# open-mmlab/PowerPaint

Hardware: AMD Instinct MI355X
Metric: inpainted images/sec @512x512, 50-step DDIM CFG, batch4/GPU (higher is better)
Workload: dtype bf16; 1 GPU; ppt-v1 SD1.5-inpaint UNet (9-ch in), 512x512, 50-step DDIM, CFG=7.5, bf16, batch=4/GPU; global_batch=4, denoise_steps=50, network_evaluations=50, parallelism=dp1 (image shards, no step collectives), hipgraph=True, weights=random init (no checkpoints offline)

## Files before the change

include/pp_hip.h:

```cpp
#ifndef PP_HIP_H_
#define PP_HIP_H_

#include <stddef.h>
#include <stdint.h>

#ifdef __cplusplus
extern "C" {
#endif

#define PP_OK 0
#define PP_ERR_BAD_ARG (-1)
#define PP_ERR_UNSUPPORTED (-2)
#define PP_ERR_LAUNCH (-3)
#define PP_ERR_WORKSPACE (-4)

#define PP_ABI_VERSION 29
#define PP_DT_F32 0
#define PP_DT_BF16 1
#define PP_DT_F16 2
int pp_abi_version(void);
const char* pp_build_id(void);
const char* pp_last_error(void);

#define PP_X_PLAIN 0
#define PP_X_CONV3X3 1
#define PP_ACT_NONE 0
#define PP_ACT_GEGLU 1
#define PP_ACT_SILU 2
#define PP_ACT_SOFTMAX80 3
#define PP_ACT_GELU 4

typedef struct PPGemmArgs {
  int32_t M, N, K;
  int32_t x_mode;
  const void* x1;
  const void* x2;
  int32_t c1, c2;
  int32_t ldx1, ldx2;
  int32_t batch, hin, win, hout, wout, stride, up;
  const void* w;
  const float* bias;
  const float* rowvec;
  int32_t ld_rowvec, rows_per_batch;
  const void* res1;
  int32_t ldres1;
  const void* res2;
  int32_t ldres2;
  float scale;
  int32_t act;
  void* out;
  int32_t ldo;
  int32_t out_f32;
  void* out_vt;
  int32_t vt_col0;
  int32_t vt_ld;
  int32_t splitk;
  int32_t tile;
  float* workspace;
  int32_t dbg;
  int32_t dtype;
  int32_t out_dup_rows;
  int32_t res1_wrap_rows;
  float* row_stats_out;
  const float* ln_stats;
  const float* ln_colsum;
  int32_t ln_tiles;
  int32_t ln_dim;
  float ln_eps;
  int32_t w_batch_stride;
  int64_t* gn_acc[2];
  int32_t gn_cg[2];
  int32_t gn_c0[2];
  int32_t gn_groups[2];
  const void* x3;
  const void* x4;
  int32_t c3;
  int32_t c4;
  const int64_t* gn_in_acc;
  const float* gn_in_gb;
  int32_t gn_in_groups;
  int32_t gn_in_silu;
  float gn_in_eps;
  int32_t gn_dup_batch;
  void* gn_next_out;
  const float* gn_next_gamma;
  const float* gn_next_beta;
  float gn_next_eps;
  int32_t gn_next_silu;
  int32_t gn_next_sub;
  int32_t gn_dup_mask;
  int32_t vec_batch_stride;
  uint64_t* tile_ctr;
  uint32_t* combine_fault;
  int32_t subpix;
  int32_t tile_group_m;
} PPGemmArgs;
#define PP_GN_SUM_SCALE 16777216.0f
#define PP_GN_SQ_SCALE 1048576.0f

#define PP_TILE_AUTO 0
#define PP_TILE_128x160 1
#define PP_TILE_64x160 2
#define PP_TILE_256x160 3

int pp_gemm_bf16(const PPGemmArgs* args, void* stream);
size_t pp_gemm_workspace_bytes(const PPGemmArgs* args);
int pp_gemm_gn_stats_ok(const PPGemmArgs* args);
int pp_conv_gn_supported(const PPGemmArgs* args);
int pp_conv_gn_preferred(const PPGemmArgs* args);
int pp_upconv_subpix_supported(int batch, int h, int w, int cin, int cout, int dtype);
int pp_upconv_subpix_supported_to(int batch, int h, int w, int hout, int wout, int cin, int cout, int dtype);
int pp_upconv_fold(const void* w, int cout, int cin, int dtype, void* out, void* stream);
int pp_gemm_gn_next_ok(const PPGemmArgs* args, int sub);
size_t pp_gemm_combine_ctr_bytes(const PPGemmArgs* args);
int pp_gemm_combine_fused(const PPGemmArgs* args);
int pp_gemm_tile_group_m(const PPGemmArgs* args);
int pp_xcd_placement_ok(void);

int pp_linear_skinny(const float* x, int rows, int K, const void* w, const float* bias, int N, float* out, int ldo,
                     int act_in, int act_out, int dtype, void* stream);

int pp_timestep_embedding(const float* t_dev, int rows, int dim, float* out, void* stream);

size_t pp_groupnorm_workspace_bytes(int batch, int hw, int C);
int pp_groupnorm_stats(const void* x1, int c1, const void* x2, int c2, int batch, int hw, int groups,
                       float* workspace, int dtype, void* stream);
int pp_groupnorm_apply(const void* x1, int c1, const void* x2, int c2, int batch, int hw, int groups, float eps,
                       const float* gamma, const float* beta, const float* workspace, int silu, void* y,
                       int dtype, void* stream);

int pp_groupnorm_apply_acc(const void* x1, int c1, const void* x2, int c2, int batch, int hw, int groups, float eps,
                           const float* gamma, const float* beta, const int64_t* acc, int silu, void* y, int dtype,
                           void* stream);
int pp_zero_u64(void* dst, long long n, void* stream);

int pp_layernorm(const void* x, int rows, int C, const float* gamma, const float* beta, float eps, void* y,
                 int dtype, void* stream);

int pp_attention_fwd(const void* q, int ldq, const void* k, int ldk, const void* vt, int ldvt, void* o, int ldo,
                     int batch, int heads, int nq, int nk, int d, float scale, int dtype, void* stream);
#define PP_ATTN_AUTO 0
#define PP_ATTN_PHASED 1
#define PP_ATTN_PIPE_Q32 2
#define PP_ATTN_PIPE_Q64 3
#define PP_ATTN_PIPE_LOG2 4
int pp_attention_log2_ok(int nq, int nk, int d);
int pp_attention_fwd_variant(const void* q, int ldq, const void* k, int ldk, const void* vt, int ldvt, void* o, int ldo,
                             int batch, int heads, int nq, int nk, int d, float scale, int dtype, int variant,
                             void* stream);
int pp_attention_tiled_ok(int h, int w, int nh, int nw, int d);
int pp_attention_fwd_tiled(const void* q, int ldq, const void* k, int ldk, const void* vt, int ldvt, void* o, int ldo,
                           int batch, int heads, int h, int w, int nh, int nw, int d, float scale, int variant,
                           int dtype, void* stream);
int pp_transpose_v(const void* v, int ld, int batch, int nk, int cols, void* vt, int ldvt, void* stream);

int pp_conv3x3_direct(const void* x, int batch, int hin, int win, int cin, const void* w, const float* bias,
                      int cout, int stride, int silu_out, const void* add, void* out, int dtype, void* stream);
int pp_conv3x3_smallcout(const void* x, int batch, int h, int w_, int cin, const void* w, const float* bias, int cout,
                         float* out_nchw, int dtype, void* stream);
int pp_gn_conv3x3_smallcout_supported(int cin, int cout, int groups);
int pp_gn_conv3x3_smallcout(const void* x, int batch, int h, int w, int cin, int groups, float eps, const float* gamma,
                            const float* beta, const int64_t* acc, const void* wgt, const float* bias, int cout,
                            float* out_nchw, int dtype, void* stream);

int pp_nchw_to_nhwc(const void* src, int src_dtype, int batch, int c, int hw, int src_batch_mod, void* dst, int ldc,
                    int c0, int dtype, void* stream);
int pp_nhwc_to_nchw(const void* src, int batch, int c, int hw, void* dst, int dst_dtype, int dtype, void* stream);
int pp_vit_patchify(const void* src, int src_dtype, int batch, int h, int w, int patch, void* dst, int cols, int ldo,
                    int dtype, void* stream);
int pp_vit_embed_ln(const void* patches, int ldp, const void* class_embedding, const void* pos, int batch, int np, int C,
                    const float* gamma, const float* beta, float eps, void* y, int dtype, void* stream);
int pp_add_bf16(const void* a, const void* b, void* out, long long n, int dtype, void* stream);

int pp_cfg_sched_step(const float* eps2, int cfg, float guidance, float* latents, float* m_prev, int n, int kind,
                      const float* coef_table, int32_t* step_dev, uint32_t* advance_ticket, void* stream);
int pp_ddim_variance_noise(float* latents, const float* noise, int n, const float* coef_table, const int32_t* step_dev,
                           void* stream);
int pp_cfg_lcm_step(const float* eps2, int cfg, float guidance, float* latents, const float* noise, int n,
                    const float* coef_table, int32_t* step_dev, uint32_t* advance_ticket, void* stream);
int pp_cfg_sigma_step(const float* eps2, int cfg, float guidance, float* latents, const float* noise, int n,
                      const float* coef_table, int32_t* step_dev, uint32_t* advance_ticket, void* stream);
int pp_cfg_ksampler_step(const float* eps2, int cfg, float guidance, float* latents, float* state, const float* noise, int n,
                         const float* coef_table, int32_t* step_dev, uint32_t* advance_ticket, void* stream);

int pp_tfront_supported(int M, int c, int rows_per_batch, int gn_groups);
int pp_tfront(const void* x, int ldx, const void* gn_acc, const float* gn_gamma, const float* gn_beta, float gn_eps, int gn_groups,
              const void* w1, const float* b1, const void* w2p, const float* cs2, const float* b2, float ln_eps, void* hs,
              int ldhs, void* qk, int ldqk, void* vt, int ldvt, int M, int c, int rows_per_batch, float q_scale, int dtype,
              void* stream);
int pp_xattn_block_supported(int M, int c, int rows_per_batch, int nctx, int heads);
int pp_xattn_fold(const void* k, int ldk, const void* vt, int ldvt, int batch, int nctx, int heads, int c, const void* wq,
                  const float* q_colsum, const float* q_bias, const void* wo, float scale, void* gt, float* gcs,
                  float* gbias, void* ht, int kperm, int dtype, void* stream);
int pp_xattn_block(const void* x, int ldx, const void* res, int ldres, const float* ln_stats, int ln_tiles, float ln_eps,
                   const void* gt, const float* gcs, const float* gbias, const void* ht, const float* bias_o, void* out,
                   int ldo, float* row_stats_out, int M, int c, int rows_per_batch, int src_wrap_rows, const void* pre_w,
                   const float* pre_b, int dtype, void* stream);

int pp_ff_fused_supported(int M, int c, int rows_per_batch);
int pp_ff_fused(const PPGemmArgs* g2, const void* w1, const float* b1, const float* cs1, const float* ln_stats, int ln_tiles,
                float ln_eps, int w2_kperm, void* stream);

int pp_latent_blend(float* latents, const float* image_latents, const float* mask, const float* noise,
                    const float* renoise_table, const int32_t* step_dev, int batch, int channels, int hw, void* stream);

int pp_step_head(const float* temb_table, const int32_t* step_dev, float* temb_out, int row_floats, const float* latents,
                 int batch, int c, int hw, int src_batch_mod, void* x_in, int ldc, int c0, int dtype, void* zero_dst,
                 long long n_zero, void* stream);
int pp_step_head_scaled(const float* temb_table, const int32_t* step_dev, float* temb_out, int row_floats, const float* latents,
                        int batch, int c, int hw, int src_batch_mod, void* x_in, int ldc, int c0, int dtype, void* zero_dst,
                        long long n_zero, const float* in_div, void* stream);
int pp_step_select_t(const float* timesteps, const int32_t* step_dev, float* t_out, void* stream);
int pp_step_advance(int32_t* step_dev, void* stream);

int pp_mask_prep(int mode, const float* a, const float* b, float* out, int batch, int c, int h, int w, int ho, int wo,
                 void* stream);

int pp_embed_splice(const void* table, const void* ext, const int32_t* src_row, void* out, int n_rows,
                    long long row_bytes, void* stream);

int pp_softmax_rows(const float* s, long long lds, int rows, int n, float scale, void* p, long long ldp, int dtype,
                    void* stream);

int pp_attention_small(const void* q, int ldq, const void* k, int ldk, const void* v, int ldv, void* o, int ldo,
                       int batch, int heads, int nq, int nk, int d, float scale, int causal, int dtype, void* stream);

#define PP_LORA_MAX_ADAPTERS 8
#define PP_LORA_MAX_RANK 128
#define PP_LORA_ROWS_PLAIN 0
#define PP_LORA_ROWS_GEGLU 1
#define PP_LORA_COLS_PLAIN 0
#define PP_LORA_COLS_IGEMM 1
#define PP_LORA_COLS_KPERM 2
#define PP_LORA_COLS_KPERM_GEGLU 3
typedef struct PPLoraMergeArgs {
  int32_t N, K;
  const float* w;
  int64_t ldw;
  int32_t n_adapters;
  int32_t rank[PP_LORA_MAX_ADAPTERS];
  float coef[PP_LORA_MAX_ADAPTERS];
  const float* up[PP_LORA_MAX_ADAPTERS];
  const float* down[PP_LORA_MAX_ADAPTERS];
  const float* gamma;
  const float* beta;
  const float* badd;
  void* out;
  int64_t ldo;
  int32_t out_rows, out_cols, out_dtype;
  int32_t row_mode, row_off;
  int32_t col_mode, col_off, taps, cin_pad;
  float* colsum;
  float* bias;
} PPLoraMergeArgs;
int pp_lora_merge(const PPLoraMergeArgs* args, void* stream);

int pp_freeu(const void* hidden, void* hidden_out, int ch, const void* skip, void* skip_out, int cs, int batch, int h, int w,
             const float* bs, int64_t* acc, int groups, int dtype, void* stream);

#define PP_IP_MAX_TOKENS 64
int pp_ip_attn_add(const void* q, int ldq, const void* k_ip, const void* v_ip, void* o, int ldo, int batch, int heads, int nq,
                   int nk, int d, float qk_scale, float ip_scale, int dtype, void* stream);

int pp_ip_attn_add_masked(const void* q, int ldq, const void* k_ip, const void* v_ip, void* o, int ldo, int batch, int heads,
                          int nq, int nk, int d, float qk_scale, float ip_scale, const float* row_w, int dtype, void* stream);

int pp_perceiver_attn(const void* q, int ldq, const void* kv_x, int ldkx, int nx, const void* kv_l, int ldkl, int nl, void* o,
                      int ldo, int batch, int heads, int nq, int d, float scale, int dtype, void* stream);

#define PP_TOME_MAX_TOKENS 16384
int pp_tome_supported(int h, int w, int C, int sx, int sy);
int pp_tome_match(const void* x, int ldx, int batch, int h, int w, int C, int sx, int sy, const void* table,
                  int table_row_stride, int table_rows, const void* row_idx, void* best_dst, void* score, int dtype,
                  void* stream);
int pp_tome_select(const void* best_dst, const void* score, int batch, int n, int nd, int r, void* pos, void* rowtok, void* seg,
                   void* lst, void* stream);
int pp_tome_merge(const void* qk, int ldqk, const void* vt, int ldvt, int batch, int n, int C, int nd, int r, const void* rowtok,
                  const void* seg, const void* lst, void* qk_out, int ldqk_out, void* vt_out, int ldvt_out, int dtype,
                  void* stream);
int pp_tome_unmerge(const void* a, int lda, const void* pos, int batch, int n, int nm, int C, void* out, int ldo, void* stream);

int pp_attn_identity_v(const void* vt, int ldvt, int batch0, int batch, int n, int C, void* out, int ldo, void* stream);
int pp_pag_combine(float* eps, int cfg, float guidance, const float* pag_table, const int32_t* step_dev, int n, void* stream);

int pp_cfg_rescale(float* eps, int segs, float guidance, const float* pag_table, const float* phi_dev, const int32_t* step_dev,
                   int batch, int per, void* stream);

int pp_conv4x4s2(const void* x, int batch, int hin, int win, int cin, const void* w, const float* bias, int cout, int relu_in,
                 void* out, int dtype, void* stream);
int pp_relu(const void* x, void* out, long long n, int dtype, void* stream);
int pp_masked_image_pack(const float* image, const float* mask, int batch, int c, int h, int w, void* out, int dtype,
                         void* stream);
int pp_mask_blend(const void* sample, const void* cond, const float* mask, void* out, int batch, int h, int w, int c,
                  int mask_h, int mask_w, int64_t* acc, int groups, int dtype, void* stream);

#ifdef __cplusplus
}
#endif
#endif
```

powerpaint_amd/_lib.py:

```python
import ctypes as C
import os

_HERE = os.path.dirname(os.path.abspath(__file__))
LIB_PATH = os.path.join(_HERE, "libpp_hip.so")
if os.environ.get("PP_LAB") == "1" and os.environ.get("PP_LIB"):
    LIB_PATH = os.path.abspath(os.environ["PP_LIB"])

PP_X_PLAIN, PP_X_CONV3X3 = 0, 1
PP_ACT_NONE, PP_ACT_GEGLU, PP_ACT_SILU, PP_ACT_SOFTMAX80, PP_ACT_GELU = 0, 1, 2, 3, 4
PP_TILE_AUTO, PP_TILE_128x160, PP_TILE_64x160, PP_TILE_256x160 = 0, 1, 2, 3
PP_DT_F32, PP_DT_BF16, PP_DT_F16 = 0, 1, 2
PP_ATTN_AUTO, PP_ATTN_PHASED, PP_ATTN_PIPE_Q32, PP_ATTN_PIPE_Q64, PP_ATTN_PIPE_LOG2 = 0, 1, 2, 3, 4
ABI_VERSION = 29
PP_ERR = {0: "PP_OK", -1: "PP_ERR_BAD_ARG", -2: "PP_ERR_UNSUPPORTED", -3: "PP_ERR_LAUNCH", -4: "PP_ERR_WORKSPACE"}

vp, i32, f32, sz = C.c_void_p, C.c_int32, C.c_float, C.c_size_t


class PPGemmArgs(C.Structure):
    _fields_ = [
        ("M", i32), ("N", i32), ("K", i32), ("x_mode", i32),
        ("x1", vp), ("x2", vp),
        ("c1", i32), ("c2", i32), ("ldx1", i32), ("ldx2", i32),
        ("batch", i32), ("hin", i32), ("win", i32), ("hout", i32), ("wout", i32), ("stride", i32), ("up", i32),
        ("w", vp), ("bias", vp), ("rowvec", vp),
        ("ld_rowvec", i32), ("rows_per_batch", i32),
        ("res1", vp), ("ldres1", i32),
        ("res2", vp), ("ldres2", i32),
        ("scale", f32), ("act", i32),
        ("out", vp), ("ldo", i32), ("out_f32", i32),
        ("out_vt", vp), ("vt_col0", i32), ("vt_ld", i32),
        ("splitk", i32), ("tile", i32),
        ("workspace", vp),
        ("dbg", i32), ("dtype", i32), ("out_dup_rows", i32), ("res1_wrap_rows", i32),
        ("row_stats_out", vp), ("ln_stats", vp), ("ln_colsum", vp),
        ("ln_tiles", i32), ("ln_dim", i32), ("ln_eps", f32), ("w_batch_stride", i32),
        ("gn_acc", vp * 2), ("gn_cg", i32 * 2), ("gn_c0", i32 * 2), ("gn_groups", i32 * 2),
        ("x3", vp), ("x4", vp), ("c3", i32), ("c4", i32),
        ("gn_in_acc", vp), ("gn_in_gb", vp), ("gn_in_groups", i32), ("gn_in_silu", i32), ("gn_in_eps", f32),
        ("gn_dup_batch", i32),
        ("gn_next_out", vp), ("gn_next_gamma", vp), ("gn_next_beta", vp), ("gn_next_eps", f32), ("gn_next_silu", i32),
        ("gn_next_sub", i32), ("gn_dup_mask", i32), ("vec_batch_stride", i32),
        ("tile_ctr", vp), ("combine_fault", vp),
        ("subpix", i32),
        ("tile_group_m", i32),
    ]


def gemm_args(dtype: int, M: int, N: int, K: int, x, w, out, x2=None, K2: int = 0, ldx=None, ldx2: int = 0, ldo: int = 0,
              ldres1: int = 0, ldres2: int = 0, rows_per_batch: int = 0, scale: float = 1.0) -> PPGemmArgs:
    a = PPGemmArgs()
    a.dtype = dtype
    a.M, a.N, a.K, a.x_mode = M, N, K + K2, PP_X_PLAIN
    a.x1, a.x2, a.c1, a.c2 = x, x2 or None, K, K2
    a.ldx1, a.ldx2 = (K if ldx is None else ldx), (ldx2 or K2)
    a.w, a.out = w, out
    a.ldo, a.ldres1, a.ldres2 = ldo or N, ldres1 or N, ldres2 or N
    a.rows_per_batch, a.scale = rows_per_batch, scale
    return a


def conv3x3_args(dtype: int, B: int, H: int, W: int, c1: int, cout: int, x, x2=None, c2: int = 0, x3=None, c3: int = 0,
                 x4=None, c4: int = 0, stride: int = 1, up: bool = False, w=None, out=None, scale: float = 1.0,
                 up_size=None) -> PPGemmArgs:
    hv, wv = (2 * H, 2 * W) if up else (H, W)
    if up_size is not None:
        if not up or stride != 1 or up_size[0] not in (2 * H - 1, 2 * H) or up_size[1] not in (2 * W - 1, 2 * W):
            raise ValueError(f"up_size {tuple(up_size)} is no nearest-resize target of a {H}x{W} source")
        hv, wv = up_size
    ho, wo = (hv - 1) // stride + 1, (wv - 1) // stride + 1
    a = PPGemmArgs()
    a.dtype = dtype
    a.M, a.N, a.K, a.x_mode = B * ho * wo, cout, 9 * (c1 + c2) + c3 + c4, PP_X_CONV3X3
    a.x1, a.x2, a.c1, a.c2 = x, x2 or None, c1, c2
    a.x3, a.x4, a.c3, a.c4 = x3 or None, x4 or None, c3, c4
    a.batch, a.hin, a.win, a.hout, a.wout, a.stride, a.up = B, H, W, ho, wo, stride, int(up)
    a.w, a.out = w, out
    a.ldo, a.ldres1, a.ldres2 = cout, cout, cout
    a.rows_per_batch, a.scale = ho * wo, scale
    return a


PP_LORA_MAX_ADAPTERS, PP_LORA_MAX_RANK = 8, 128
PP_LORA_ROWS_PLAIN, PP_LORA_ROWS_GEGLU = 0, 1
PP_TOME_MAX_TOKENS = 16384
PP_IP_MAX_TOKENS = 64
PP_LORA_COLS_PLAIN, PP_LORA_COLS_IGEMM, PP_LORA_COLS_KPERM, PP_LORA_COLS_KPERM_GEGLU = 0, 1, 2, 3


class PPLoraMergeArgs(C.Structure):
    _fields_ = [
        ("N", i32), ("K", i32), ("w", vp), ("ldw", C.c_int64), ("n_adapters", i32),
        ("rank", i32 * PP_LORA_MAX_ADAPTERS), ("coef", f32 * PP_LORA_MAX_ADAPTERS),
        ("up", vp * PP_LORA_MAX_ADAPTERS), ("down", vp * PP_LORA_MAX_ADAPTERS),
        ("gamma", vp), ("beta", vp), ("badd", vp),
        ("out", vp), ("ldo", C.c_int64), ("out_rows", i32), ("out_cols", i32), ("out_dtype", i32),
        ("row_mode", i32), ("row_off", i32), ("col_mode", i32), ("col_off", i32), ("taps", i32), ("cin_pad", i32),
        ("colsum", vp), ("bias", vp),
    ]


SIGNATURES = {
    "pp_abi_version": (C.c_int, []),
    "pp_last_error": (C.c_char_p, []),
    "pp_build_id": (C.c_char_p, []),
    "pp_gemm_bf16": (C.c_int, [C.POINTER(PPGemmArgs), vp]),
    "pp_gemm_workspace_bytes": (sz, [C.POINTER(PPGemmArgs)]),
    "pp_linear_skinny": (C.c_int, [vp, C.c_int, C.c_int, vp, vp, C.c_int, vp, C.c_int, C.c_int, C.c_int, C.c_int, vp]),
    "pp_timestep_embedding": (C.c_int, [vp, C.c_int, C.c_int, vp, vp]),
    "pp_groupnorm_workspace_bytes": (sz, [C.c_int, C.c_int, C.c_int]),
    "pp_gemm_gn_stats_ok": (C.c_int, [C.POINTER(PPGemmArgs)]),
    "pp_conv_gn_supported": (C.c_int, [C.POINTER(PPGemmArgs)]),
    "pp_conv_gn_preferred": (C.c_int, [C.POINTER(PPGemmArgs)]),
    "pp_gemm_gn_next_ok": (C.c_int, [C.POINTER(PPGemmArgs), C.c_int]),
    "pp_upconv_subpix_supported": (C.c_int, [C.c_int] * 6),
    "pp_upconv_subpix_supported_to": (C.c_int, [C.c_int] * 8),
    "pp_upconv_fold": (C.c_int, [vp, C.c_int, C.c_int, C.c_int, vp, vp]),
    "pp_gemm_combine_ctr_bytes": (sz, [C.POINTER(PPGemmArgs)]),
    "pp_gemm_combine_fused": (C.c_int, [C.POINTER(PPGemmArgs)]),
    "pp_gemm_tile_group_m": (C.c_int, [C.POINTER(PPGemmArgs)]),
    "pp_xcd_placement_ok": (C.c_int, []),
    "pp_groupnorm_apply_acc": (C.c_int, [vp, C.c_int, vp, C.c_int, C.c_int, C.c_int, C.c_int, f32, vp, vp, vp, C.c_int, vp,
                                         C.c_int, vp]),
    "pp_zero_u64": (C.c_int, [vp, C.c_longlong, vp]),
    "pp_embed_splice": (C.c_int, [vp, vp, vp, vp, C.c_int, C.c_longlong, vp]),
    "pp_attention_small": (C.c_int, [vp, C.c_int, vp, C.c_int, vp, C.c_int, vp, C.c_int, C.c_int, C.c_int, C.c_int,
                                     C.c_int, C.c_int, f32, C.c_int, C.c_int, vp]),
    "pp_softmax_rows": (C.c_int, [vp, C.c_longlong, C.c_int, C.c_int, f32, vp, C.c_longlong, C.c_int, vp]),
    "pp_groupnorm_stats": (C.c_int, [vp, C.c_int, vp, C.c_int, C.c_int, C.c_int, C.c_int, vp, C.c_int, vp]),
    "pp_groupnorm_apply": (C.c_int, [vp, C.c_int, vp, C.c_int, C.c_int, C.c_int, C.c_int, f32, vp, vp, vp, C.c_int, vp,
                                     C.c_int, vp]),
    "pp_layernorm": (C.c_int, [vp, C.c_int, C.c_int, vp, vp, f32, vp, C.c_int, vp]),
    "pp_attention_fwd": (C.c_int, [vp, C.c_int, vp, C.c_int, vp, C.c_int, vp, C.c_int, C.c_int, C.c_int, C.c_int,
                                   C.c_int, C.c_int, f32, C.c_int, vp]),
    "pp_attention_fwd_variant": (C.c_int, [vp, C.c_int, vp, C.c_int, vp, C.c_int, vp, C.c_int, C.c_int, C.c_int, C.c_int,
                                           C.c_int, C.c_int, f32, C.c_int, C.c_int, vp]),
    "pp_attention_tiled_ok": (C.c_int, [C.c_int] * 5),
    "pp_attention_fwd_tiled": (C.c_int, [vp, C.c_int, vp, C.c_int, vp, C.c_int, vp, C.c_int, C.c_int, C.c_int, C.c_int,
                                         C.c_int, C.c_int, C.c_int, C.c_int, f32, C.c_int, C.c_int, vp]),
    "pp_transpose_v": (C.c_int, [vp, C.c_int, C.c_int, C.c_int, C.c_int, vp, C.c_int, vp]),
    "pp_conv3x3_direct": (C.c_int, [vp, C.c_int, C.c_int, C.c_int, C.c_int, vp, vp, C.c_int, C.c_int, C.c_int, vp,
                                    vp, C.c_int, vp]),
    "pp_conv3x3_smallcout": (C.c_int, [vp, C.c_int, C.c_int, C.c_int, C.c_int, vp, vp, C.c_int, vp, C.c_int, vp]),
    "pp_nchw_to_nhwc": (C.c_int, [vp, C.c_int, C.c_int, C.c_int, C.c_int, C.c_int, vp, C.c_int, C.c_int, C.c_int, vp]),
    "pp_nhwc_to_nchw": (C.c_int, [vp, C.c_int, C.c_int, C.c_int, vp, C.c_int, C.c_int, vp]),
    "pp_vit_patchify": (C.c_int, [vp, C.c_int, C.c_int, C.c_int, C.c_int, C.c_int, vp, C.c_int, C.c_int, C.c_int, vp]),
    "pp_vit_embed_ln": (C.c_int, [vp, C.c_int, vp, vp, C.c_int, C.c_int, C.c_int, vp, vp, f32, vp, C.c_int, vp]),
    "pp_add_bf16": (C.c_int, [vp, vp, vp, C.c_longlong, C.c_int, vp]),
    "pp_cfg_sched_step": (C.c_int, [vp, C.c_int, f32, vp, vp, C.c_int, C.c_int, vp, vp, vp, vp]),
    "pp_step_select_t": (C.c_int, [vp, vp, vp, vp]),
    "pp_ddim_variance_noise": (C.c_int, [vp, vp, C.c_int, vp, vp, vp]),
    "pp_cfg_lcm_step": (C.c_int, [vp, C.c_int, f32, vp, vp, C.c_int, vp, vp, vp, vp]),
    "pp_cfg_sigma_step": (C.c_int, [vp, C.c_int, f32, vp, vp, C.c_int, vp, vp, vp, vp]),
    "pp_cfg_ksampler_step": (C.c_int, [vp, C.c_int, f32, vp, vp, vp, C.c_int, vp, vp, vp, vp]),
    "pp_latent_blend": (C.c_int, [vp, vp, vp, vp, vp, vp, C.c_int, C.c_int, C.c_int, vp]),
    "pp_gn_conv3x3_smallcout_supported": (C.c_int, [C.c_int] * 3),
    "pp_gn_conv3x3_smallcout": (C.c_int, [vp, C.c_int, C.c_int, C.c_int, C.c_int, C.c_int, C.c_float, vp, vp, vp, vp, vp,
                                          C.c_int, vp, C.c_int, vp]),
    "pp_tfront_supported": (C.c_int, [C.c_int] * 4),
    "pp_tfront": (C.c_int, [vp, C.c_int, vp, vp, vp, C.c_float, C.c_int, vp, vp, vp, vp, vp, C.c_float, vp, C.c_int, vp, C.c_int,
                            vp, C.c_int, C.c_int, C.c_int, C.c_int, C.c_float, C.c_int, vp]),
    "pp_attention_log2_ok": (C.c_int, [C.c_int] * 3),
    "pp_xattn_block_supported": (C.c_int, [C.c_int] * 5),
    "pp_xattn_fold": (C.c_int, [vp, C.c_int, vp, C.c_int, C.c_int, C.c_int, C.c_int, C.c_int, vp, vp, vp, vp, C.c_float,
                                vp, vp, vp, vp, C.c_int, C.c_int, vp]),
    "pp_xattn_block": (C.c_int, [vp, C.c_int, vp, C.c_int, vp, C.c_int, C.c_float, vp, vp, vp, vp, vp, vp, C.c_int, vp,
                                 C.c_int, C.c_int, C.c_int, C.c_int, vp, vp, C.c_int, vp]),
    "pp_ff_fused_supported": (C.c_int, [C.c_int] * 3),
    "pp_ff_fused": (C.c_int, [C.POINTER(PPGemmArgs), vp, vp, vp, vp, C.c_int, C.c_float, C.c_int, vp]),
    "pp_step_head": (C.c_int, [vp, vp, vp, C.c_int, vp, C.c_int, C.c_int, C.c_int, C.c_int, vp, C.c_int, C.c_int, C.c_int, vp,
                              C.c_longlong, vp]),
    "pp_step_head_scaled": (C.c_int, [vp, vp, vp, C.c_int, vp, C.c_int, C.c_int, C.c_int, C.c_int, vp, C.c_int, C.c_int, C.c_int,
                                     vp, C.c_longlong, vp, vp]),
    "pp_step_advance": (C.c_int, [vp, vp]),
    "pp_lora_merge": (C.c_int, [C.POINTER(PPLoraMergeArgs), vp]),
    "pp_freeu": (C.c_int, [vp, vp, C.c_int, vp, vp, C.c_int, C.c_int, C.c_int, C.c_int, vp, vp, C.c_int, C.c_int, vp]),
    "pp_mask_prep": (C.c_int, [C.c_int, vp, vp, vp, C.c_int, C.c_int, C.c_int, C.c_int, C.c_int, C.c_int, vp]),
    "pp_ip_attn_add": (C.c_int, [vp, C.c_int, vp, vp, vp, C.c_int, C.c_int, C.c_int, C.c_int, C.c_int, C.c_int, f32, f32,
                                 C.c_int, vp]),
    "pp_ip_attn_add_masked": (C.c_int, [vp, C.c_int, vp, vp, vp, C.c_int, C.c_int, C.c_int, C.c_int, C.c_int, C.c_int, f32, f32,
                                        vp, C.c_int, vp]),
    "pp_perceiver_attn": (C.c_int, [vp, C.c_int, vp, C.c_int, C.c_int, vp, C.c_int, C.c_int, vp, C.c_int, C.c_int, C.c_int,
                                    C.c_int, C.c_int, f32, C.c_int, vp]),
    "pp_tome_supported": (C.c_int, [C.c_int] * 5),
    "pp_tome_match": (C.c_int, [vp, C.c_int, C.c_int, C.c_int, C.c_int, C.c_int, C.c_int, C.c_int, vp, C.c_int, C.c_int, vp, vp,
                                vp, C.c_int, vp]),
    "pp_tome_select": (C.c_int, [vp, vp, C.c_int, C.c_int, C.c_int, C.c_int, vp, vp, vp, vp, vp]),
    "pp_tome_merge": (C.c_int, [vp, C.c_int, vp, C.c_int, C.c_int, C.c_int, C.c_int, C.c_int, C.c_int, vp, vp, vp, vp, C.c_int,
                                vp, C.c_int, C.c_int, vp]),
    "pp_tome_unmerge": (C.c_int, [vp, C.c_int, vp, C.c_int, C.c_int, C.c_int, C.c_int, vp, C.c_int, vp]),
    "pp_attn_identity_v": (C.c_int, [vp, C.c_int, C.c_int, C.c_int, C.c_int, C.c_int, vp, C.c_int, vp]),
    "pp_pag_combine": (C.c_int, [vp, C.c_int, f32, vp, vp, C.c_int, vp]),
    "pp_cfg_rescale": (C.c_int, [vp, C.c_int, f32, vp, vp, vp, C.c_int, C.c_int, vp]),
    "pp_conv4x4s2": (C.c_int, [vp, C.c_int, C.c_int, C.c_int, C.c_int, vp, vp, C.c_int, C.c_int, vp, C.c_int, vp]),
    "pp_relu": (C.c_int, [vp, vp, C.c_longlong, C.c_int, vp]),
    "pp_masked_image_pack": (C.c_int, [vp, vp, C.c_int, C.c_int, C.c_int, C.c_int, vp, C.c_int, vp]),
    "pp_mask_blend": (C.c_int, [vp, vp, vp, vp, C.c_int, C.c_int, C.c_int, C.c_int, C.c_int, C.c_int, vp, C.c_int, C.c_int, vp]),
}

_lib = None


class PPError(RuntimeError):
    pass


def lib():
    global _lib
    if _lib is None:
        if not os.path.exists(LIB_PATH):
            raise PPError(
                f"{LIB_PATH} not found: the HIP extension is not built. Run `python -c 'import __graft_entry__ as g; "
                f"g.build()'` (or `make -C powerpaint_amd/csrc`). There is no CPU/PyTorch fallback.")
        l = C.CDLL(LIB_PATH)
        for name, (res, args) in SIGNATURES.items():
            fn = getattr(l, name)
            fn.restype = res
            fn.argtypes = args
        if l.pp_abi_version() != ABI_VERSION:
            raise PPError("libpp_hip.so ABI version mismatch")
        _lib = l
    return _lib


def dtype_code(dtype) -> int:
    import torch
    if dtype == torch.bfloat16:
        return PP_DT_BF16
    if dtype == torch.float16:
        return PP_DT_F16
    raise PPError(f"the HIP path computes in bf16 or fp16 (fp32 accumulate), not {dtype}")


def build_id() -> str:
    return lib().pp_build_id().decode()


def check(rc: int, what: str = ""):
    if rc != 0:
        msg = lib().pp_last_error().decode() if rc == -3 else ""
        raise PPError(f"{what} failed: {PP_ERR.get(rc, rc)} {msg}")
```

powerpaint_amd/csrc/conv_gn.hip:

```cpp
#include <type_traits>
#include <utility>

#include "pp_common.h"
#include "gemm_gn.h"
#include "gemm_combine.h"

namespace {

typedef __attribute__((address_space(3))) void* cg_lds_t;

constexpr int CG_T = 512, CG_BN = 160, CG_NI = 5;
constexpr int CG_WP = 3;
constexpr int CG_HPW_MAX = 6;
constexpr int CG_HALO_PX = 384;
constexpr int CG_HALO = CG_HALO_PX * 128;
constexpr int CG_WST = CG_BN * 128;
constexpr int CG_WOFF = 2 * CG_HALO;
constexpr int CG_TAB = CG_WOFF + 3 * CG_WST;
constexpr int CG_T_STATS = CG_TAB;
constexpr int CG_T_ZERO = CG_TAB + 256;
constexpr int CG_T_GB = CG_TAB + 1024;
constexpr int CG_T_SCSH = CG_TAB + 3072;
constexpr int CG_LDS = CG_TAB + 3584;
static_assert(CG_LDS <= 160 * 1024, "LDS budget");

struct CGDerived {
  int tiles_m, tiles_n, group_m;
  int nch1, nch;
  int ntail3, ntail;
  int hp;
  int cg;
  float inv_cg;
};

template <int... I, class F>
PP_DEVINL void cg_static_for_impl(std::integer_sequence<int, I...>, F&& f) { (f(std::integral_constant<int, I>{}), ...); }
template <int N, class F>
PP_DEVINL void cg_static_for(F&& f) { cg_static_for_impl(std::make_integer_sequence<int, N>{}, f); }

template <int BM, int HPW, bool PP, int NMODE, int EDT>
__global__ void __launch_bounds__(CG_T, 2) pp_conv_gn_kernel(const PPGemmArgs a, const CGDerived d) {
  using E = E16<EDT>;
  typedef typename E::v8 v8_t;
  constexpr int T = CG_T, WN = 2, MI = BM / 64, NI = CG_NI, BN = CG_BN;
  constexpr int CG_HPW = HPW;
  constexpr bool SUBPIX = NMODE == 4;
  static_assert(!SUBPIX || PP, "the sub-pixel form has the ping-pong loop only");
  constexpr bool NORM = NMODE != 2 && !SUBPIX;
  constexpr bool NREAD = NMODE == 0 || NMODE == 3;
  static_assert(HPW >= 2 && HPW <= CG_HPW_MAX, "halo strips per wave");
  constexpr int XP2 = BM / 64;
  constexpr int P2 = XP2 + CG_WP;
  constexpr int ST2 = BM * 128;
  constexpr int EPI_ROWS = 64, EPI_LD = BN * 4 + 16;
  constexpr int RS_OFF = EPI_ROWS * EPI_LD + BM * 8;
  static_assert(3 * ST2 <= 2 * CG_HALO, "tail stages live in the halo buffers");
  static_assert(MI * 16 <= EPI_ROWS && EPI_ROWS % (MI * 16) == 0, "wave rows vs epilogue pass");

  extern __shared__ __attribute__((aligned(16))) char smem[];

  const int tid = threadIdx.x;
  const int lane = tid & 63;
  const int wave = __builtin_amdgcn_readfirstlane(tid >> 6);
  const int wm = wave >> 1, wn = wave & 1;
  const int grp = wave >> 2;

  int lid;
  {
    const int nwg = gridDim.x, bid = blockIdx.x;
    const int q = nwg >> 3, r = nwg & 7, xcd = bid & 7, idx = bid >> 3;
    lid = (xcd < r ? xcd * (q + 1) : r * (q + 1) + (xcd - r) * q) + idx;
  }
  const int par = SUBPIX ? (lid & 3) : 0, pa = par >> 1, pb = par & 1;
  if constexpr (SUBPIX) lid >>= 2;
  int tile_m, tile_n;
  pp_tile_decode(lid, d.tiles_m, d.tiles_n, d.group_m, &tile_m, &tile_n);
  const int m_blk = tile_m * BM, n_blk = tile_n * BN;
  const int split = blockIdx.y, splits = gridDim.y;
  const int ch_b = split * d.nch / splits, ch_e = (split + 1) * d.nch / splits;
  const int tk_b = split * d.ntail / splits, tk_e = (split + 1) * d.ntail / splits;

  const int Wd = a.wout, Hd = a.hout, HW = Hd * Wd;
  const int HWs = a.hin * a.win;
  const int bimg = m_blk / HW;
  const int y0 = (m_blk - bimg * HW) / Wd;
  const int ctot = a.c1 + a.c2;
  const uint32_t wbytes = (uint32_t)a.N * (uint32_t)a.K * 2u;
  const void* const wmat = SUBPIX ? (const void*)((const char*)a.w + (size_t)par * wbytes) : a.w;

  const int lrow = lane >> 3;
  const int kslot = (lane & 7) ^ lrow;

  int vw[CG_WP], wlds[CG_WP];
#pragma unroll
  for (int i = 0; i < CG_WP; ++i) {
    const int strip = (wave * 8 + i * 64 < BN) ? i : i - 1;
    const int n = n_blk + wave * 8 + lrow + strip * 64;
    vw[i] = (n < a.N) ? (n * a.K + kslot * 8) * 2 : (int)PP_OOB;
    wlds[i] = (wave * 8 + strip * 64) * 128;
  }
  int hpix[CG_HPW];
#pragma unroll
  for (int j = 0; j < CG_HPW; ++j) {
    const int hp = (wave + 8 * j) * 8 + lrow;
    const int hr = hp / Wd, hx = hp - hr * Wd;
    const int iy = y0 + hr - 1;
    hpix[j] = (hp < d.hp && iy >= 0 && iy < Hd) ? (a.up ? bimg * HWs + (iy >> 1) * a.win + (hx >> 1) : bimg * HW + iy * Wd + hx) : -1;
  }
  const int r16 = lane & 15, g = lane >> 4;
  const int fsw = r16 & 7;
  const int wrow0 = wn * (NI * 16) + r16;
  const int rt0 = wm * (MI * 16) + r16;
  unsigned edge = 0u;
#pragma unroll
  for (int mi = 0; mi < MI; ++mi) {
    const int lx = (rt0 + mi * 16) % Wd;
    if (lx == 0) edge |= 1u << mi;
    if (lx == Wd - 1) edge |= 1u << (8 + mi);
  }

  f32x4_t acc[NI][MI];
#pragma unroll
  for (int ni = 0; ni < NI; ++ni)
#pragma unroll
    for (int mi = 0; mi < MI; ++mi) acc[ni][mi] = f32x4_t{0.f, 0.f, 0.f, 0.f};

  auto mfma_all = [&](const v8_t (&wf)[2][NI], const v8_t (&xf)[2][MI]) __attribute__((always_inline)) {
#pragma unroll
    for (int ks = 0; ks < 2; ++ks)
#pragma unroll
      for (int ni = 0; ni < NI; ++ni)
#pragma unroll
        for (int mi = 0; mi < MI; ++mi) acc[ni][mi] = E::mfma16(wf[ks][ni], xf[ks][mi], acc[ni][mi]);
  };

  if (ch_b < ch_e) {
    auto issue_gb = [&](int c, int gbuf, bool live) __attribute__((always_inline)) {
      const __amdgpu_buffer_rsrc_t rs = make_rsrc(a.gn_in_gb, (NORM && live) ? (uint32_t)ctot * 8u : 0u);
      const int vo = lane < 32 ? lane * 16 : (int)PP_OOB;
      __builtin_amdgcn_raw_ptr_buffer_load_lds(rs, (cg_lds_t)(smem + CG_T_GB + gbuf * 1024), 16, vo, c * 512, 0, 0);
    };
    auto compute_scsh = [&](int c, int gbuf) __attribute__((always_inline)) {
      const char* gp = smem + CG_T_GB + gbuf * 1024 + kslot * 64;
      const f32x2_t* st = reinterpret_cast<const f32x2_t*>(smem + CG_T_STATS);
#pragma unroll
      for (int q = 0; q < 4; ++q) {
        const f32x4_t gbv = *reinterpret_cast<const f32x4_t*>(gp + q * 16);
        f32x4_t o;
#pragma unroll
        for (int h = 0; h < 2; ++h) {
          const int ch = c * 64 + kslot * 8 + 2 * q + h;
          const int gi = min((int)(((float)ch + 0.5f) * d.inv_cg), 31);
          const f32x2_t mr = st[gi];
          const float sv = mr[1] * gbv[2 * h];
          o[2 * h] = sv;
          o[2 * h + 1] = gbv[2 * h + 1] - mr[0] * sv;
        }
        if (lrow == 0) *reinterpret_cast<f32x4_t*>(smem + CG_T_SCSH + kslot * 64 + q * 16) = o;
      }
      asm volatile("s_waitcnt lgkmcnt(0)" ::: "memory");
    };
    auto norm_piece = [&](int hbuf, int j) __attribute__((always_inline)) {
      char* p = smem + hbuf * CG_HALO + (wave + 8 * j) * 1024 + lane * 16;
      if (hpix[j] >= 0) {
        const u32x4_t v = *reinterpret_cast<const u32x4_t*>(p);
        float r[8];
#pragma unroll
        for (int q = 0; q < 4; ++q) {
          const f32x4_t ss = *reinterpret_cast<const f32x4_t*>(smem + CG_T_SCSH + kslot * 64 + q * 16);
          r[2 * q] = E::lo(v[q]) * ss[0] + ss[1];
          r[2 * q + 1] = E::hi(v[q]) * ss[2] + ss[3];
        }
#pragma unroll
        for (int e = 0; e < 8; ++e)
          r[e] = r[e] * __builtin_amdgcn_rcpf(1.0f + __builtin_amdgcn_exp2f(r[e] * -1.44269504088896340736f));
        u32x4_t o;
#pragma unroll
        for (int q = 0; q < 4; ++q) o[q] = E::pack2(r[2 * q], r[2 * q + 1]);
        *reinterpret_cast<u32x4_t*>(p) = o;
      }
    };

    auto norm_math = [&](const u32x4_t v, uint32_t vmask) __attribute__((always_inline)) -> u32x4_t {
      u32x4_t o;
#pragma unroll
      for (int q = 0; q < 4; ++q) {
        const f32x4_t ss = *reinterpret_cast<const f32x4_t*>(smem + CG_T_SCSH + kslot * 64 + q * 16);
        float r0 = E::lo(v[q]) * ss[0] + ss[1];
        float r1 = E::hi(v[q]) * ss[2] + ss[3];
        const float e0 = __builtin_amdgcn_exp2f(r0 * -1.44269504088896340736f);
        const float e1 = __builtin_amdgcn_exp2f(r1 * -1.44269504088896340736f);
        r0 *= __builtin_amdgcn_rcpf(1.0f + e0);
        r1 *= __builtin_amdgcn_rcpf(1.0f + e1);
        o[q] = E::pack2(r0, r1) & vmask;
      }
      return o;
    };

    __amdgpu_buffer_rsrc_t rs_h = make_rsrc(a.x1, 0u);
    int hsoff = 0, hcsrc = 0;
    auto halo_source = [&](int c, bool live) __attribute__((always_inline)) {
      const bool first = c < d.nch1;
      int csrc;
      if (first) {
        csrc = a.c1;
        rs_h = make_rsrc(a.x1, live ? (uint32_t)a.batch * (uint32_t)HWs * (uint32_t)a.c1 * 2u : 0u);
        hsoff = c * 128;
      } else {
        csrc = a.c2;
        rs_h = make_rsrc(a.x2 ? a.x2 : a.x1, (live && a.x2) ? (uint32_t)a.batch * (uint32_t)HWs * (uint32_t)a.c2 * 2u : 0u);
        hsoff = (c - d.nch1) * 128;
      }
      hcsrc = csrc;
    };
    auto issue_halo_piece = [&](int hbuf, int j) __attribute__((always_inline)) {
      const int vo = hpix[j] >= 0 ? (hpix[j] * hcsrc + kslot * 8) * 2 : (int)PP_OOB;
      __builtin_amdgcn_raw_ptr_buffer_load_lds(rs_h, (cg_lds_t)(smem + hbuf * CG_HALO + (wave + 8 * j) * 1024), 16, vo,
                                               hsoff, 0, 0);
    };
    auto issue_w_piece = [&](const __amdgpu_buffer_rsrc_t rs, int stage, int i, int sow) __attribute__((always_inline)) {
      const int vo = vw[i], lo = wlds[i];
      __builtin_amdgcn_raw_ptr_buffer_load_lds(rs, (cg_lds_t)(smem + CG_WOFF + stage * CG_WST + lo), 16, vo, sow, 0, 0);
    };

    {
      const __amdgpu_buffer_rsrc_t rsw = make_rsrc(wmat, wbytes);
#pragma unroll
      for (int i = 0; i < CG_WP; ++i) issue_w_piece(rsw, 0, i, (0 * ctot + ch_b * 64) * 2);
#pragma unroll
      for (int i = 0; i < CG_WP; ++i) issue_w_piece(rsw, 1, i, (1 * ctot + ch_b * 64) * 2);
      halo_source(ch_b, true);
#pragma unroll
      for (int j = 0; j < CG_HPW; ++j) issue_halo_piece(0, j);
      issue_gb(ch_b, 0, true);
    }
    if (NORM && tid < a.gn_in_groups) {
      const long long* ap = reinterpret_cast<const long long*>(a.gn_in_acc) + ((size_t)bimg * a.gn_in_groups + tid) * 2;
      const double s = (double)ap[0] * (1.0 / (double)PP_GN_SUM_SCALE);
      const double q = (double)ap[1] * (1.0 / (double)PP_GN_SQ_SCALE);
      const double n = (double)HW * (double)d.cg;
      const double mean = s / n;
      double var = q / n - mean * mean;
      if (var < 0.0) var = 0.0;
      reinterpret_cast<f32x2_t*>(smem + CG_T_STATS)[tid] = f32x2_t{(float)mean, (float)(1.0 / sqrt(var + (double)a.gn_in_eps))};
    }
    if (tid < 32) reinterpret_cast<float*>(smem + CG_T_ZERO)[tid] = 0.f;
    asm volatile("s_waitcnt vmcnt(0) lgkmcnt(0)\n\ts_barrier" ::: "memory");
    if constexpr (NORM) {
      compute_scsh(ch_b, 0);
#pragma unroll
      for (int j = 0; j < CG_HPW; ++j) norm_piece(0, j);
    }
    asm volatile("s_waitcnt lgkmcnt(0)\n\ts_barrier" ::: "memory");
    if (PP && grp == 1) asm volatile("s_barrier" ::: "memory");

    int hb = 0;
    if constexpr (SUBPIX) {
      int st = 0;
      const int tap00 = pa * Wd + pb - 1;
      const unsigned em0 = pb == 0 ? (edge & 0xffu) : 0u, em1 = pb == 1 ? (edge >> 8) : 0u;
#pragma unroll 1
      for (int c = ch_b; c < ch_e; ++c) {
        const bool nxt = c + 1 < ch_e;
        halo_source(c + 1, nxt);
        const __amdgpu_buffer_rsrc_t rsw_same = make_rsrc(wmat, wbytes);
        const __amdgpu_buffer_rsrc_t rsw_next = make_rsrc(wmat, nxt ? wbytes : 0u);
        const int hoff = hb * CG_HALO;
        const int hbn = hb ^ 1;
        int Wl = Wd;
        asm volatile("" : "+s"(Wl));

        cg_static_for<4>([&](auto TT) __attribute__((always_inline)) {
          constexpr int t = decltype(TT)::value;
          constexpr auto NXT = [](int tt) constexpr { return tt > 2 ? 0 : (2 * tt + 2 <= CG_HPW ? 2 : 2 * tt + 1 <= CG_HPW ? 1 : 0); };
          constexpr int NX = NXT(t);
          const int st_w = st == 0 ? 2 : st - 1;
          const __amdgpu_buffer_rsrc_t rsw = t + 2 <= 3 ? rsw_same : rsw_next;
          const int sow = t + 2 <= 3 ? ((t + 2) * ctot + c * 64) * 2 : ((t + 2 - 4) * ctot + (c + 1) * 64) * 2;

          asm volatile("s_barrier" ::: "memory");
          const char* ws = smem + CG_WOFF + st * CG_WST;
          const int hp0 = rt0 + tap00 + (t / 2) * Wl + (t % 2);
          const int xbase = hoff + (hp0 << 7) + ((g ^ (hp0 & 7)) << 4);
          const unsigned em = t % 2 == 0 ? em0 : em1;
          v8_t wf[2][NI], xf[2][MI];
          constexpr int NR = NI + MI, NPC = CG_WP + NX;
#pragma unroll
          for (int r = 0; r < NR; ++r) {
            if (r < NI) {
              const int ni = r < NI ? r : 0;
              const char* pw = ws + (wrow0 + ni * 16) * 128;
              wf[0][ni] = *reinterpret_cast<const v8_t*>(pw + ((g ^ fsw) << 4));
              wf[1][ni] = *reinterpret_cast<const v8_t*>(pw + (((4 + g) ^ fsw) << 4));
            } else {
              const int mi = r >= NI ? r - NI : 0;
              int o0 = xbase + mi * 2048;
              o0 = (em >> mi) & 1u ? CG_T_ZERO : o0;
              xf[0][mi] = *reinterpret_cast<const v8_t*>(smem + o0);
              xf[1][mi] = *reinterpret_cast<const v8_t*>(smem + (o0 ^ 64));
            }
#pragma unroll
            for (int k = 0; k < NPC; ++k)
              if (((k + 1) * NR + NPC) / (NPC + 1) == r + 1) {
                __builtin_amdgcn_sched_barrier(0);
                if (k < CG_WP) issue_w_piece(rsw, st_w, k < CG_WP ? k : 0, sow);
                else issue_halo_piece(hbn, 2 * t + (k - CG_WP < 2 ? k - CG_WP : 0));
                __builtin_amdgcn_sched_barrier(0);
              }
          }
          constexpr int V = (t == 3 ? 0 : NXT((t + 3) % 4)) + CG_WP + NX;
          asm volatile("s_waitcnt vmcnt(%0) lgkmcnt(0)\n\ts_barrier" ::"n"(V) : "memory");
          __builtin_amdgcn_sched_barrier(0);
          __builtin_amdgcn_s_setprio(1);
          mfma_all(wf, xf);
          __builtin_amdgcn_s_setprio(0);
          __builtin_amdgcn_sched_barrier(0);
          st = st == 2 ? 0 : st + 1;
        });
        hb ^= 1;
      }
    } else {
  #pragma unroll 1
      for (int c = ch_b; c < ch_e; ++c) {
        const bool nxt = c + 1 < ch_e;
        halo_source(c + 1, nxt);
        const __amdgpu_buffer_rsrc_t rsw_same = make_rsrc(wmat, wbytes);
        const __amdgpu_buffer_rsrc_t rsw_next = make_rsrc(wmat, nxt ? wbytes : 0u);
        const int hoff = hb * CG_HALO;
        const int hbn = hb ^ 1;
        int Wl = Wd;
        asm volatile("" : "+s"(Wl));

        cg_static_for<9>([&](auto TT) __attribute__((always_inline)) {
          constexpr int t = decltype(TT)::value;
          constexpr int st_r = t % 3, st_w = (t + 2) % 3;
          constexpr auto NXT = [](int tt) constexpr {
            const int nh = tt > 2 ? 0 : (2 * tt + 2 <= CG_HPW ? 2 : 2 * tt + 1 <= CG_HPW ? 1 : 0);
            return nh + (tt == 0 ? 1 : 0);
          };
          constexpr int NX = NXT(t);
          const __amdgpu_buffer_rsrc_t rsw = t + 2 <= 8 ? rsw_same : rsw_next;
          const int sow = t + 2 <= 8 ? ((t + 2) * ctot + c * 64) * 2 : ((t + 2 - 9) * ctot + (c + 1) * 64) * 2;

          if constexpr (PP) {
            asm volatile("s_barrier" ::: "memory");
          } else {
            constexpr int V = NXT((t + 7) % 9) + CG_WP + NXT((t + 8) % 9);
            asm volatile("s_waitcnt vmcnt(%0) lgkmcnt(0)\n\ts_barrier" ::"n"(V) : "memory");
          }
          constexpr bool NT = NORM && t >= 3 && t - 3 < CG_HPW;
          char* const np = smem + hbn * CG_HALO + (wave + 8 * (NT ? t - 3 : 0)) * 1024 + lane * 16;
          u32x4_t nv = {0u, 0u, 0u, 0u};
          f32x4_t ss0 = {0.f, 0.f, 0.f, 0.f}, ss1 = {0.f, 0.f, 0.f, 0.f};
          if constexpr (NT) {
            if constexpr (t == 3) compute_scsh(c + 1, hbn);
            if constexpr (NREAD) norm_piece(hbn, t - 3);
            else {
              nv = *reinterpret_cast<const u32x4_t*>(np);
              ss0 = *reinterpret_cast<const f32x4_t*>(smem + CG_T_SCSH + kslot * 64);
              ss1 = *reinterpret_cast<const f32x4_t*>(smem + CG_T_SCSH + kslot * 64 + 16);
            }
            if constexpr (NREAD) __builtin_amdgcn_sched_barrier(0);
          }
          const char* ws = smem + CG_WOFF + st_r * CG_WST;
          const int hp0 = rt0 + (t / 3) * Wl + (t % 3) - 1;
          const int xbase = hoff + (hp0 << 7) + ((g ^ (hp0 & 7)) << 4);
          v8_t wf[2][NI], xf[2][MI];
          constexpr int NR = NI + MI, NPC = CG_WP + NX;
  #pragma unroll
          for (int r = 0; r < NR; ++r) {
            if (r < NI) {
              const int ni = r < NI ? r : 0;
              const char* pw = ws + (wrow0 + ni * 16) * 128;
              wf[0][ni] = *reinterpret_cast<const v8_t*>(pw + ((g ^ fsw) << 4));
              wf[1][ni] = *reinterpret_cast<const v8_t*>(pw + (((4 + g) ^ fsw) << 4));
            } else {
              const int mi = r >= NI ? r - NI : 0;
              int o0 = xbase + mi * 2048;
              if constexpr (t % 3 == 0) o0 = (edge >> mi) & 1u ? CG_T_ZERO : o0;
              if constexpr (t % 3 == 2) o0 = (edge >> (8 + mi)) & 1u ? CG_T_ZERO : o0;
              xf[0][mi] = *reinterpret_cast<const v8_t*>(smem + o0);
              xf[1][mi] = *reinterpret_cast<const v8_t*>(smem + (o0 ^ 64));
            }
  #pragma unroll
            for (int k = 0; k < NPC; ++k)
              if (((k + 1) * NR + NPC) / (NPC + 1) == r + 1) {
                __builtin_amdgcn_sched_barrier(0);
                if (k < CG_WP) issue_w_piece(rsw, st_w, k < CG_WP ? k : 0, sow);
                else if (t == 0 && k == NPC - 1) issue_gb(c + 1, hbn, nxt);
                else issue_halo_piece(hbn, 2 * t + (k - CG_WP < 2 ? k - CG_WP : 0));
                __builtin_amdgcn_sched_barrier(0);
              }
          }
          if constexpr (PP) {
            constexpr int V = NXT((t + 8) % 9) + CG_WP + NX;
            asm volatile("s_waitcnt vmcnt(%0) lgkmcnt(0)\n\ts_barrier" ::"n"(V) : "memory");
          }
          __builtin_amdgcn_sched_barrier(0);
          if constexpr (NMODE != 3) __builtin_amdgcn_s_setprio(1);
          if constexpr (NT && NMODE == 1) {
            constexpr int NM = 2 * MI * NI, NG = 41;
            const uint32_t vmask = ~(uint32_t)(hpix[NT ? t - 3 : 0] >> 31);
            const char* const sp = smem + CG_T_SCSH + kslot * 64;
            float xa[4], ea[4];
            u32x4_t no;
            auto micro = [&](auto GG) __attribute__((always_inline)) {
              constexpr int g = decltype(GG)::value;
              if constexpr (g == 40) {
                *reinterpret_cast<u32x4_t*>(np) = no;
              } else {
                constexpr int h = g / 20, gg = g % 20, p0 = 2 * h, p1 = 2 * h + 1;
                if constexpr (gg == 0) { xa[0] = E::lo(nv[p0]); xa[1] = E::hi(nv[p0]); }
                if constexpr (gg == 1) { xa[2] = E::lo(nv[p1]); xa[3] = E::hi(nv[p1]); }
                if constexpr (gg == 2) { xa[0] = __builtin_fmaf(xa[0], ss0[0], ss0[1]); xa[1] = __builtin_fmaf(xa[1], ss0[2], ss0[3]); }
                if constexpr (gg == 3) { xa[2] = __builtin_fmaf(xa[2], ss1[0], ss1[1]); xa[3] = __builtin_fmaf(xa[3], ss1[2], ss1[3]); }
                if constexpr (gg == 4) { ea[0] = xa[0] * -1.44269504088896340736f; ea[1] = xa[1] * -1.44269504088896340736f; }
                if constexpr (gg == 5) { ea[2] = xa[2] * -1.44269504088896340736f; ea[3] = xa[3] * -1.44269504088896340736f; }
                if constexpr (gg == 6) {
                  ea[0] = __builtin_amdgcn_exp2f(ea[0]);
                  if constexpr (h == 0) ss0 = *reinterpret_cast<const f32x4_t*>(sp + 32);
                }
                if constexpr (gg == 7) {
                  ea[1] = __builtin_amdgcn_exp2f(ea[1]);
                  if constexpr (h == 0) ss1 = *reinterpret_cast<const f32x4_t*>(sp + 48);
                }
                if constexpr (gg == 8) ea[2] = __builtin_amdgcn_exp2f(ea[2]);
                if constexpr (gg == 9) ea[3] = __builtin_amdgcn_exp2f(ea[3]);
                if constexpr (gg == 10) { ea[0] += 1.0f; ea[1] += 1.0f; }
                if constexpr (gg == 11) { ea[2] += 1.0f; ea[3] += 1.0f; }
                if constexpr (gg == 12) ea[0] = __builtin_amdgcn_rcpf(ea[0]);
                if constexpr (gg == 13) ea[1] = __builtin_amdgcn_rcpf(ea[1]);
                if constexpr (gg == 14) ea[2] = __builtin_amdgcn_rcpf(ea[2]);
                if constexpr (gg == 15) ea[3] = __builtin_amdgcn_rcpf(ea[3]);
                if constexpr (gg == 16) { xa[0] *= ea[0]; xa[1] *= ea[1]; }
                if constexpr (gg == 17) { xa[2] *= ea[2]; xa[3] *= ea[3]; }
                if constexpr (gg == 18) no[p0] = E::pack2(xa[0], xa[1]) & vmask;
                if constexpr (gg == 19) no[p1] = E::pack2(xa[2], xa[3]) & vmask;
              }
            };
            cg_static_for<NM>([&](auto II) __attribute__((always_inline)) {
              constexpr int i = decltype(II)::value;
              constexpr int ks = i / (NI * MI), ni = (i / MI) % NI, mi = i % MI;
              acc[ni][mi] = E::mfma16(wf[ks][ni], xf[ks][mi], acc[ni][mi]);
              __builtin_amdgcn_sched_barrier(0);
              constexpr int G0 = i * NG / NM, G1 = (i + 1) * NG / NM;
              cg_static_for<G1 - G0>([&](auto JJ) __attribute__((always_inline)) {
                micro(std::integral_constant<int, G0 + decltype(JJ)::value>{});
              });
              __builtin_amdgcn_sched_barrier(0);
            });
          } else {
            mfma_all(wf, xf);
          }
          if constexpr (NMODE != 3) __builtin_amdgcn_s_setprio(0);
          __builtin_amdgcn_sched_barrier(0);
        });
        hb ^= 1;
      }
    }
    if (PP && grp == 0) asm volatile("s_barrier" ::: "memory");
    asm volatile("s_waitcnt vmcnt(0)" ::: "memory");
  }

  if (tk_b < tk_e) {
    asm volatile("s_waitcnt lgkmcnt(0)\n\ts_barrier" ::: "memory");
    const int mrow = m_blk + wave * 8 + lrow;
    const uint32_t xb3 = (uint32_t)a.M * (uint32_t)a.c3 * 2u, xb4 = a.x4 ? (uint32_t)a.M * (uint32_t)a.c4 * 2u : 0u;
    auto issue2 = [&](int kt, int stage) __attribute__((always_inline)) {
      const bool live = kt < tk_e;
      const bool first = kt < d.ntail3;
      const __amdgpu_buffer_rsrc_t rsx = first ? make_rsrc(a.x3, live ? xb3 : 0u) : make_rsrc(a.x4 ? a.x4 : a.x3, live ? xb4 : 0u);
      const int sox = (first ? kt : kt - d.ntail3) * 128;
      const int csrc = first ? a.c3 : a.c4;
      const __amdgpu_buffer_rsrc_t rsw = make_rsrc(a.w, live ? wbytes : 0u);
      const int sow = (9 * ctot + kt * 64) * 2;
#pragma unroll
      for (int i = 0; i < XP2; ++i) {
        const int m = mrow + i * 64;
        const int vo = m < a.M ? (m * csrc + kslot * 8) * 2 : (int)PP_OOB;
        __builtin_amdgcn_raw_ptr_buffer_load_lds(rsx, (cg_lds_t)(smem + stage * ST2 + (wave * 8 + i * 64) * 128), 16, vo, sox,
                                                 0, 0);
      }
#pragma unroll
      for (int i = 0; i < CG_WP; ++i) {
        const int vo = vw[i], lo = wlds[i];
        __builtin_amdgcn_raw_ptr_buffer_load_lds(rsw, (cg_lds_t)(smem + CG_WOFF + stage * CG_WST + lo), 16, vo, sow, 0, 0);
      }
    };
    issue2(tk_b, 0);
    issue2(tk_b + 1, 1);
    const int xrow0 = wm * (MI * 16) + r16;
    int stage = 0;
#pragma unroll 1
    for (int kt = tk_b; kt < tk_e; ++kt) {
      asm volatile("s_waitcnt vmcnt(%0)\n\ts_barrier" ::"n"(P2) : "memory");
      int nstage = stage + 2;
      if (nstage >= 3) nstage -= 3;
      issue2(kt + 2, nstage);
      const char* xs = smem + stage * ST2;
      const char* ws = smem + CG_WOFF + stage * CG_WST;
      v8_t wf[2][NI], xf[2][MI];
#pragma unroll
      for (int ks = 0; ks < 2; ++ks) {
        const int so = ((ks * 4 + g) ^ fsw) << 4;
#pragma unroll
        for (int ni = 0; ni < NI; ++ni) wf[ks][ni] = *reinterpret_cast<const v8_t*>(ws + (wrow0 + ni * 16) * 128 + so);
#pragma unroll
        for (int mi = 0; mi < MI; ++mi) xf[ks][mi] = *reinterpret_cast<const v8_t*>(xs + (xrow0 + mi * 16) * 128 + so);
      }
      __builtin_amdgcn_sched_barrier(0);
      __builtin_amdgcn_s_setprio(1);
      mfma_all(wf, xf);
      __builtin_amdgcn_s_setprio(0);
      stage = stage + 1 == 3 ? 0 : stage + 1;
    }
    asm volatile("s_waitcnt vmcnt(0)" ::: "memory");
  }

  auto out_row = [&](int m) __attribute__((always_inline)) -> size_t {
    const int l = m - bimg * HW, i = l / Wd, j = l - i * Wd;
    return (size_t)bimg * 4u * (size_t)HW + (size_t)((2 * i + pa) * 2 * Wd + 2 * j + pb);
  };
  const bool splitk = splits > 1;
  const bool gns = !splitk && (a.gn_acc[0] || a.gn_acc[1]);
  const int my_pass = (wm * (MI * 16)) / EPI_ROWS;
  const int my_row0 = (wm * (MI * 16)) % EPI_ROWS;
  float gcs[8], gcq[8];
#pragma unroll
  for (int jj = 0; jj < 8; ++jj) { gcs[jj] = 0.f; gcq[jj] = 0.f; }
  constexpr int EC = BN / 8, ER = T / EC, EP = (EPI_ROWS + ER - 1) / ER;
  const int c8 = tid % EC, r0 = tid / EC;
  const int n = n_blk + c8 * 8;
#pragma unroll 1
  for (int pass = 0; pass < BM / EPI_ROWS; ++pass) {
    asm volatile("s_waitcnt lgkmcnt(0)\n\ts_barrier" ::: "memory");
    if (my_pass == pass) {
#pragma unroll
      for (int mi = 0; mi < MI; ++mi)
#pragma unroll
        for (int ni = 0; ni < NI; ++ni)
          *reinterpret_cast<f32x4_t*>(smem + (my_row0 + mi * 16 + r16) * EPI_LD + (wn * (NI * 16) + ni * 16 + 4 * g) * 4) =
              acc[ni][mi];
    }
    asm volatile("s_waitcnt lgkmcnt(0)\n\ts_barrier" ::: "memory");
    const int m0 = m_blk + pass * EPI_ROWS;
    if (r0 < ER && n < a.N) {
      if (splitk) {
#pragma unroll
        for (int j = 0; j < EP; ++j) {
          const int row = r0 + j * ER, m = m0 + row;
          if (row < EPI_ROWS && m < a.M) {
            float* wsp = a.workspace + ((size_t)split * a.M + m) * a.N + n;
            *reinterpret_cast<f32x4_t*>(wsp) = *reinterpret_cast<const f32x4_t*>(smem + row * EPI_LD + c8 * 32);
            *reinterpret_cast<f32x4_t*>(wsp + 4) = *reinterpret_cast<const f32x4_t*>(smem + row * EPI_LD + c8 * 32 + 16);
          }
        }
      } else {
        u32x4_t r1[EP], r2[EP];
#pragma unroll
        for (int j = 0; j < EP; ++j) {
          const int row = r0 + j * ER, m = m0 + row;
          const bool ok = row < EPI_ROWS && m < a.M;
          const size_t m1 = SUBPIX ? out_row(m) : (size_t)((a.res1_wrap_rows > 0 && m >= a.res1_wrap_rows) ? m - a.res1_wrap_rows : m);
          const size_t m2 = SUBPIX ? out_row(m) : (size_t)m;
          r1[j] = (ok && a.res1) ? *reinterpret_cast<const u32x4_t*>((const uint16_t*)a.res1 + m1 * a.ldres1 + n)
                                 : u32x4_t{0u, 0u, 0u, 0u};
          r2[j] = (ok && a.res2) ? *reinterpret_cast<const u32x4_t*>((const uint16_t*)a.res2 + m2 * a.ldres2 + n)
                                 : u32x4_t{0u, 0u, 0u, 0u};
        }
        f32x4_t bs0 = {0.f, 0.f, 0.f, 0.f}, bs1 = {0.f, 0.f, 0.f, 0.f};
        if (a.bias) {
          bs0 = *reinterpret_cast<const f32x4_t*>(a.bias + n);
          bs1 = *reinterpret_cast<const f32x4_t*>(a.bias + n + 4);
        }
        if (a.rowvec) {
          const float* rv = a.rowvec + (size_t)(m_blk / a.rows_per_batch) * a.ld_rowvec + n;
          bs0 += *reinterpret_cast<const f32x4_t*>(rv);
          bs1 += *reinterpret_cast<const f32x4_t*>(rv + 4);
        }
#pragma unroll
        for (int j = 0; j < EP; ++j) {
          const int row = r0 + j * ER, m = m0 + row;
          if (row < EPI_ROWS && m < a.M) {
            f32x4_t v0 = *reinterpret_cast<const f32x4_t*>(smem + row * EPI_LD + c8 * 32);
            f32x4_t v1 = *reinterpret_cast<const f32x4_t*>(smem + row * EPI_LD + c8 * 32 + 16);
            v0 += bs0;
            v1 += bs1;
            v0 *= a.scale;
            v1 *= a.scale;
            v0[0] += E::lo(r1[j][0]) + E::lo(r2[j][0]); v0[1] += E::hi(r1[j][0]) + E::hi(r2[j][0]);
            v0[2] += E::lo(r1[j][1]) + E::lo(r2[j][1]); v0[3] += E::hi(r1[j][1]) + E::hi(r2[j][1]);
            v1[0] += E::lo(r1[j][2]) + E::lo(r2[j][2]); v1[1] += E::hi(r1[j][2]) + E::hi(r2[j][2]);
            v1[2] += E::lo(r1[j][3]) + E::lo(r2[j][3]); v1[3] += E::hi(r1[j][3]) + E::hi(r2[j][3]);
            u32x4_t o;
            o[0] = E::pack2(v0[0], v0[1]); o[1] = E::pack2(v0[2], v0[3]);
            o[2] = E::pack2(v1[0], v1[1]); o[3] = E::pack2(v1[2], v1[3]);
            *reinterpret_cast<u32x4_t*>((uint16_t*)a.out + (SUBPIX ? out_row(m) : (size_t)m) * a.ldo + n) = o;
            if (gns) {
#pragma unroll
              for (int jj = 0; jj < 4; ++jj) {
                const float lo = E::lo(o[jj]), hi = E::hi(o[jj]);
                gcs[2 * jj] += lo; gcq[2 * jj] += lo * lo;
                gcs[2 * jj + 1] += hi; gcq[2 * jj + 1] += hi * hi;
              }
            }
          }
        }
      }
    }
  }
  if (gns) {
    unsigned long long* slots = reinterpret_cast<unsigned long long*>(smem + RS_OFF);
    if (tid < 2 * GN_SLOTS * 2) slots[tid] = 0ull;
    asm volatile("s_waitcnt lgkmcnt(0)\n\ts_barrier" ::: "memory");
    if (r0 < ER && n < a.N) {
      float* dstp = reinterpret_cast<float*>(smem) + ((size_t)r0 * BN + c8 * 8) * 2;
#pragma unroll
      for (int jj = 0; jj < 4; ++jj)
        *reinterpret_cast<f32x4_t*>(dstp + 4 * jj) = f32x4_t{gcs[2 * jj], gcq[2 * jj], gcs[2 * jj + 1], gcq[2 * jj + 1]};
    }
    asm volatile("s_waitcnt lgkmcnt(0)\n\ts_barrier" ::: "memory");
    const int ncols = min(BN, a.N - n_blk);
    if (tid < ncols) {
      float sm = 0.f, sq = 0.f;
#pragma unroll 5
      for (int r = 0; r < ER; ++r) {
        const f32x2_t v = *reinterpret_cast<const f32x2_t*>(smem + ((size_t)r * BN + tid) * 8);
        sm += v[0];
        sq += v[1];
      }
      gn_column(a, slots, n_blk, tid, sm, sq);
    }
    asm volatile("s_waitcnt lgkmcnt(0)\n\ts_barrier" ::: "memory");
    gn_flush(a, slots, m_blk, n_blk, ncols, tid);
  }
  if (splitk && a.tile_ctr) {
    static_assert(fc_lds_bytes(BM) <= CG_LDS, "fused combine staging must fit in the kernel's LDS");
    splitk_fused_combine<BM, T, EDT>(a, smem, m_blk, n_blk, blockIdx.x, blockIdx.y, splits, tid);
  }
}

bool cg_shape_ok(const PPGemmArgs& a, int bm) {
  const int hw = a.hout * a.wout;
  return bm % a.wout == 0 && hw % bm == 0 && bm + 2 * a.wout <= CG_HALO_PX;
}

bool cg_geometry_ok(const PPGemmArgs& a) {
  if (a.x_mode != PP_X_CONV3X3 || !pp_dt_ok(a.dtype)) return false;
  if (a.stride != 1 || a.wout < 8 || (a.wout & 7)) return false;
  if (a.up ? (a.hout != 2 * a.hin || a.wout != 2 * a.win) : (a.hin != a.hout || a.win != a.wout)) return false;
  const int ctot = a.c1 + a.c2;
  if (a.c1 <= 0 || a.c1 % 64 || a.c2 % 64 || (a.c2 > 0 && !a.x2)) return false;
  if (a.c3 < 0 || a.c4 < 0 || a.c3 % 64 || a.c4 % 64 || (a.c3 > 0 && !a.x3) || (a.c4 > 0 && (!a.x4 || a.c3 == 0))) return false;
  if (a.K != (a.subpix ? 4 : 9) * ctot + a.c3 + a.c4 || a.M != a.batch * a.hout * a.wout || a.M <= 0 || a.N <= 0) return false;
  if (a.N % 8 || a.ldo % 8 || a.out_f32 || a.out_vt || a.act != PP_ACT_NONE || a.ln_stats || a.row_stats_out) return false;
  if ((a.res1 && a.ldres1 % 8) || (a.res2 && a.ldres2 % 8)) return false;
  if (a.rows_per_batch != a.hout * a.wout || a.out_dup_rows > 0 || a.w_batch_stride > 0 || a.vec_batch_stride > 0) return false;
  if ((uint64_t)a.batch * a.hin * a.win * (uint64_t)(a.c1 > a.c2 ? a.c1 : a.c2) * 2u >= 0x80000000ull) return false;
  if ((uint64_t)a.N * (uint64_t)a.K * 2u >= 0x80000000ull) return false;
  if ((uint64_t)a.M * (uint64_t)(a.c3 > a.c4 ? a.c3 : a.c4) * 2u >= 0x80000000ull) return false;
  for (int k = 0; k < 2; ++k)
    if (a.gn_acc[k] && (a.gn_cg[k] < 8 || a.gn_groups[k] <= 0 || a.gn_c0[k] < 0)) return false;
  return cg_shape_ok(a, 256) || cg_shape_ok(a, 128) || cg_shape_ok(a, 64);
}

bool cg_fused_ok(const PPGemmArgs& a) {
  if (!a.gn_in_acc || !a.gn_in_gb || a.up || a.subpix || !cg_geometry_ok(a)) return false;
  if (a.gn_in_silu != 1 || a.gn_in_groups <= 0 || a.gn_in_groups > 32) return false;
  return (a.c1 + a.c2) % a.gn_in_groups == 0;
}

bool cg_raw_ok(const PPGemmArgs& a) {
  static const int min_w = pp_lab_env("PP_CONV_RAW", 16);
  if (a.gn_in_acc || a.gn_in_gb || a.subpix || a.tile != PP_TILE_AUTO || min_w <= 0 || a.wout < min_w) return false;
  return cg_geometry_ok(a);
}

bool cg_subpix_ok(const PPGemmArgs& a) {
  if (a.subpix != 1 || a.up || a.gn_in_acc || a.gn_in_gb || a.c2 || a.c3 || a.c4 || a.splitk > 1) return false;
  if (a.res1_wrap_rows > 0 || a.gn_next_out || a.gn_dup_mask) return false;
  return cg_geometry_ok(a);
}

CGChoice cg_choose_subpix(const PPGemmArgs& a) {
  const int tn = (a.N + 159) / 160;
  const int want = a.tile == PP_TILE_256x160 ? 256 : a.tile == PP_TILE_128x160 ? 128 : a.tile == PP_TILE_64x160 ? 64 : 0;
  if (want && cg_shape_ok(a, want)) return CGChoice{want, 1};
  for (int bm = 256; bm >= 64; bm >>= 1)
    if (cg_shape_ok(a, bm) && 4 * (a.M / bm) * tn >= 224) return CGChoice{bm, 1};
  return CGChoice{cg_shape_ok(a, 256) ? 256 : cg_shape_ok(a, 128) ? 128 : 64, 1};
}

CGChoice cg_choose(const PPGemmArgs& a) {
  const int tn = (a.N + 159) / 160;
  auto tiles = [&](int bm) { return (a.M / bm) * tn; };
  CGChoice c{0, 1};
  const int want = a.tile == PP_TILE_256x160 ? 256 : a.tile == PP_TILE_128x160 ? 128 : a.tile == PP_TILE_64x160 ? 64 : 0;
  const int nch0 = (a.c1 + a.c2) / 64;
  static const int sk2_from = pp_lab_env("PP_CONV_GN_SK2", 12);
#ifdef PP_LAB
  static const int w16 = pp_lab_env("PP_CONV_GN_W16", 0);
  if (w16 > 0 && a.wout == 16 && !want && a.splitk <= 0 && cg_shape_ok(a, w16 / 10)) {
    c.bm = w16 / 10;
    c.splitk = w16 % 10;
    if (c.splitk > nch0) c.splitk = nch0;
    return c;
  }
#endif
  if (want && cg_shape_ok(a, want)) c.bm = want;
  else if (cg_shape_ok(a, 256) && tiles(256) >= 224) c.bm = 256;
  else if (sk2_from > 0 && nch0 >= sk2_from && a.splitk <= 0 && cg_shape_ok(a, 256) && tiles(256) * 2 >= 224 &&
           tiles(256) < 224 && cg_shape_ok(a, 128) && tiles(128) >= 224) {
    c.bm = 256;
    c.splitk = 2;
    return c;
  }
  else if (cg_shape_ok(a, 128) && tiles(128) >= 224) c.bm = 128;
  else if (cg_shape_ok(a, 256) && cg_shape_ok(a, 128) && tiles(256) * 4 <= 256 && nch0 <= 10 && a.splitk <= 0) c.bm = 128;
  else if (cg_shape_ok(a, 256)) c.bm = 256;
  else if (cg_shape_ok(a, 128)) c.bm = 128;
  else c.bm = 64;
  const int nch = (a.c1 + a.c2) / 64;
  int sk = 1;
  while (tiles(c.bm) * sk * 2 <= 256 && nch / (sk * 2) >= 2 && sk < 8) sk *= 2;
  c.splitk = a.splitk > 0 ? a.splitk : sk;
  if (c.splitk > 8) c.splitk = 8;
  if (c.splitk > nch) c.splitk = nch;
  return c;
}

template <int BM, int HPW, bool PP, int NMODE, int EDT>
int cg_launch(const PPGemmArgs& a, int splitk, int group_m, hipStream_t st) {
  auto kern = pp_conv_gn_kernel<BM, HPW, PP, NMODE, EDT>;
  if (pp_func_lds(reinterpret_cast<const void*>(kern), CG_LDS, "hipFuncSetAttribute(conv_gn)") != PP_OK) return PP_ERR_LAUNCH;
  CGDerived d;
  d.tiles_m = a.M / BM;
  d.tiles_n = (a.N + CG_BN - 1) / CG_BN;
  d.group_m = group_m < 1 ? 1 : group_m > d.tiles_m ? d.tiles_m : group_m;
  d.nch1 = a.c1 / 64;
  d.nch = (a.c1 + a.c2) / 64;
  d.ntail3 = a.c3 / 64;
  d.ntail = (a.c3 + a.c4) / 64;
  d.hp = BM + 2 * a.wout;
  d.cg = a.gn_in_groups > 0 ? (a.c1 + a.c2) / a.gn_in_groups : 1;
  d.inv_cg = 1.0f / (float)d.cg;
  hipLaunchKernelGGL(kern, dim3(d.tiles_m * d.tiles_n * (NMODE == 4 ? 4 : 1), splitk, 1), dim3(CG_T), CG_LDS, st, a, d);
  PP_CHECK_LAUNCH("pp_conv_gn_kernel");
  return PP_OK;
}

template <int BM, bool PP, int NMODE, int EDT>
int cg_launch_hpw(const PPGemmArgs& a, int splitk, int group_m, hipStream_t st) {
  const int need = (BM + 2 * a.wout + 63) / 64;
  if constexpr (BM == 256) {
    if (need <= 5) return cg_launch<256, 5, PP, NMODE, EDT>(a, splitk, group_m, st);
    return cg_launch<256, 6, PP, NMODE, EDT>(a, splitk, group_m, st);
  } else if constexpr (BM == 128) {
    if (need <= 3) return cg_launch<128, 3, PP, NMODE, EDT>(a, splitk, group_m, st);
    if (need <= 4) return cg_launch<128, 4, PP, NMODE, EDT>(a, splitk, group_m, st);
    return cg_launch<128, 6, PP, NMODE, EDT>(a, splitk, group_m, st);
  } else {
    if (need <= 2) return cg_launch<64, 2, PP, NMODE, EDT>(a, splitk, group_m, st);
    return cg_launch<64, 3, PP, NMODE, EDT>(a, splitk, group_m, st);
  }
}

template <int EDT>
int cg_dispatch(const PPGemmArgs& a, const CGChoice& c, hipStream_t st) {
#ifdef PP_LAB
  static const int pp = pp_lab_env("PP_CONV_GN_PP", 1), nm = pp_lab_env("PP_CONV_GN_NMODE", 1);
  if (!pp || nm != 1) {
#define CG_CASE(BM_)                                                                        \
    case BM_:                                                                               \
      if (!pp) return cg_launch_hpw<BM_, false, 1, EDT>(a, c.splitk, c.group_m, st);                   \
      if (nm == 0) return cg_launch_hpw<BM_, true, 0, EDT>(a, c.splitk, c.group_m, st);                \
      if (nm == 2) return cg_launch_hpw<BM_, true, 2, EDT>(a, c.splitk, c.group_m, st);                \
      return cg_launch_hpw<BM_, true, 3, EDT>(a, c.splitk, c.group_m, st);
    switch (c.bm) {
      CG_CASE(256)
      CG_CASE(128)
      default:
      CG_CASE(64)
    }
#undef CG_CASE
  }
#endif
  if (a.subpix) {
    switch (c.bm) {
      case 256: return cg_launch_hpw<256, true, 4, EDT>(a, 1, c.group_m, st);
      case 128: return cg_launch_hpw<128, true, 4, EDT>(a, 1, c.group_m, st);
      default: return cg_launch_hpw<64, true, 4, EDT>(a, 1, c.group_m, st);
    }
  }
  if (!a.gn_in_acc) {
    switch (c.bm) {
      case 256: return cg_launch_hpw<256, true, 2, EDT>(a, c.splitk, c.group_m, st);
      case 128: return cg_launch_hpw<128, true, 2, EDT>(a, c.splitk, c.group_m, st);
      default: return cg_launch_hpw<64, true, 2, EDT>(a, c.splitk, c.group_m, st);
    }
  }
  switch (c.bm) {
    case 256: return cg_launch_hpw<256, true, 1, EDT>(a, c.splitk, c.group_m, st);
    case 128: return cg_launch_hpw<128, true, 1, EDT>(a, c.splitk, c.group_m, st);
    default: return cg_launch_hpw<64, true, 1, EDT>(a, c.splitk, c.group_m, st);
  }
}

}

int pp_conv_gn_form(const PPGemmArgs& a, CGChoice* c) {
  if (a.x_mode != PP_X_CONV3X3) return 0;
  if (a.subpix) {
    if (!cg_subpix_ok(a)) return PP_ERR_UNSUPPORTED;
    *c = cg_choose_subpix(a);
    return 1;
  }
  if (a.gn_in_acc) {
    if (!cg_fused_ok(a)) return PP_ERR_UNSUPPORTED;
  } else if (!cg_raw_ok(a)) {
    return 0;
  }
  *c = cg_choose(a);
  return 1;
}
void pp_conv_gn_operand_bytes(const PPGemmArgs& a, int bm, long long* panel, long long* strip) {
  const long long px = bm + 2 * a.wout;
  *panel = (a.up ? (px + 3) / 4 : px) * (a.c1 + a.c2) * 2ll + (long long)bm * (a.c3 + a.c4) * 2ll;
  *strip = (long long)(a.N < CG_BN ? a.N : CG_BN) * a.K * 2ll * (a.subpix ? 4 : 1);
}
int pp_conv_gn_run(const PPGemmArgs& a, const CGChoice& c, hipStream_t st) {
  if (c.splitk > 1 && !a.workspace) return PP_ERR_WORKSPACE;
  return a.dtype == PP_DT_F16 ? cg_dispatch<PP_DT_F16>(a, c, st) : cg_dispatch<PP_DT_BF16>(a, c, st);
}

extern "C" int pp_conv_gn_supported(const PPGemmArgs* args) {
  if (!args) return 0;
  return cg_fused_ok(*args) ? 1 : cg_raw_ok(*args) ? 2 : 0;
}

extern "C" int pp_upconv_subpix_supported(int batch, int h, int w, int cin, int cout, int dtype) {
  if (batch <= 0 || h <= 0 || w <= 0 || cin <= 0 || cout <= 0) return 0;
  PPGemmArgs a = {};
  a.x_mode = PP_X_CONV3X3;
  a.dtype = dtype;
  a.batch = batch;
  a.hin = a.hout = h;
  a.win = a.wout = w;
  a.stride = 1;
  a.c1 = cin;
  a.M = batch * h * w;
  a.N = cout;
  a.K = 4 * cin;
  a.ldo = a.ldres1 = a.ldres2 = cout;
  a.rows_per_batch = h * w;
  a.subpix = 1;
  if ((uint64_t)batch * h * w * 4u * (uint64_t)cout * 2u >= (1ull << 40)) return 0;
  if (!cg_subpix_ok(a)) return 0;
  return w >= 16 ? 2 : 1;
}

extern "C" int pp_upconv_subpix_supported_to(int batch, int h, int w, int hout, int wout, int cin, int cout, int dtype) {
  if (hout != 2 * h || wout != 2 * w) return 0;
  return pp_upconv_subpix_supported(batch, h, w, cin, cout, dtype);
}

extern "C" int pp_conv_gn_preferred(const PPGemmArgs* args) {
  if (!args || !cg_fused_ok(*args)) return 0;
  const PPGemmArgs& a = *args;
  const int nch = (a.c1 + a.c2) / 64;
  int cls;
  if (a.win >= 64) cls = 1;
  else if (a.win == 32) cls = (nch <= 5 && a.c2 == 0) ? 2 : 8;
  else if (a.win == 16) cls = 4;
  else cls = a.win < 16 ? 16 : 8;
  static const int mask = pp_lab_env("PP_CONV_GN_ROUTE", 0);
  return (mask & cls) ? 1 : 0;
}
```

powerpaint_amd/csrc/pp_common.h:

```cpp
#pragma once
#include <hip/hip_runtime.h>
#include <stdint.h>
#include <stdlib.h>

#include "pp_hip.h"
#include "tile_order.h"

typedef __attribute__((ext_vector_type(8))) __bf16 bf16x8_t;
typedef __attribute__((ext_vector_type(4))) float f32x4_t;
typedef __attribute__((ext_vector_type(16))) float f32x16_t;
typedef __attribute__((ext_vector_type(4))) uint32_t u32x4_t;
typedef __attribute__((ext_vector_type(2))) uint32_t u32x2_t;

#define PP_DEVINL __device__ __forceinline__

PP_DEVINL float bf2f(uint16_t v) { return __uint_as_float(((uint32_t)v) << 16); }
PP_DEVINL uint16_t f2bf(float f) {
  __bf16 b = (__bf16)f;
  return __builtin_bit_cast(uint16_t, b);
}
typedef __attribute__((ext_vector_type(2))) float f32x2_t;
typedef __attribute__((ext_vector_type(2))) __bf16 bf16x2_t;
PP_DEVINL uint32_t pack2bf(float lo, float hi) {
  const f32x2_t v = {lo, hi};
  return __builtin_bit_cast(uint32_t, __builtin_convertvector(v, bf16x2_t));
}
PP_DEVINL float bflo(uint32_t u) { return __uint_as_float(u << 16); }
PP_DEVINL float bfhi(uint32_t u) { return __uint_as_float(u & 0xffff0000u); }

typedef __attribute__((ext_vector_type(8))) _Float16 f16x8_t;
typedef __attribute__((ext_vector_type(2))) _Float16 f16x2_t;
template <int DT>
struct E16;
template <>
struct E16<PP_DT_BF16> {
  typedef bf16x8_t v8;
  static PP_DEVINL float to_f(uint16_t v) { return bf2f(v); }
  static PP_DEVINL uint16_t from_f(float f) { return f2bf(f); }
  static PP_DEVINL float lo(uint32_t u) { return bflo(u); }
  static PP_DEVINL float hi(uint32_t u) { return bfhi(u); }
  static PP_DEVINL uint32_t pack2(float lo, float hi) { return pack2bf(lo, hi); }
  static PP_DEVINL f32x4_t mfma16(v8 a, v8 b, f32x4_t c) { return __builtin_amdgcn_mfma_f32_16x16x32_bf16(a, b, c, 0, 0, 0); }
  static PP_DEVINL f32x16_t mfma32(v8 a, v8 b, f32x16_t c) { return __builtin_amdgcn_mfma_f32_32x32x16_bf16(a, b, c, 0, 0, 0); }
  static PP_DEVINL f32x16_t mfma32(v8 a, v8 b, f32x16_t c, int, int, int) { return mfma32(a, b, c); }
  static PP_DEVINL f32x4_t mfma16(v8 a, v8 b, f32x4_t c, int, int, int) { return mfma16(a, b, c); }
};
template <>
struct E16<PP_DT_F16> {
  typedef f16x8_t v8;
  static PP_DEVINL float to_f(uint16_t v) { return (float)__builtin_bit_cast(_Float16, v); }
  static PP_DEVINL uint16_t from_f(float f) { return __builtin_bit_cast(uint16_t, (_Float16)f); }
  static PP_DEVINL float lo(uint32_t u) { return to_f((uint16_t)(u & 0xffffu)); }
  static PP_DEVINL float hi(uint32_t u) { return to_f((uint16_t)(u >> 16)); }
  static PP_DEVINL uint32_t pack2(float lo, float hi) {
    const f32x2_t v = {lo, hi};
    return __builtin_bit_cast(uint32_t, __builtin_convertvector(v, f16x2_t));
  }
  static PP_DEVINL f32x4_t mfma16(v8 a, v8 b, f32x4_t c) { return __builtin_amdgcn_mfma_f32_16x16x32_f16(a, b, c, 0, 0, 0); }
  static PP_DEVINL f32x16_t mfma32(v8 a, v8 b, f32x16_t c) { return __builtin_amdgcn_mfma_f32_32x32x16_f16(a, b, c, 0, 0, 0); }
  static PP_DEVINL f32x16_t mfma32(v8 a, v8 b, f32x16_t c, int, int, int) { return mfma32(a, b, c); }
  static PP_DEVINL f32x4_t mfma16(v8 a, v8 b, f32x4_t c, int, int, int) { return mfma16(a, b, c); }
};
#define PP_DT_SWITCH(DTV, ...)                    \
  do {                                            \
    if ((DTV) == PP_DT_F16) {                     \
      constexpr int EDT = PP_DT_F16;               \
      __VA_ARGS__;                                \
    } else {                                      \
      constexpr int EDT = PP_DT_BF16;             \
      __VA_ARGS__;                                \
    }                                             \
  } while (0)
inline bool pp_dt_ok(int dt) { return dt == PP_DT_BF16 || dt == PP_DT_F16; }

PP_DEVINL float silu_f(float x) { return x / (1.0f + __expf(-x)); }
PP_DEVINL float silu_fast_f(float x) { return x * __builtin_amdgcn_rcpf(1.0f + __builtin_amdgcn_exp2f(x * -1.44269504088896340736f)); }
PP_DEVINL float gelu_erf_f(float x) { return 0.5f * x * (1.0f + erff(x * 0.70710678118654752440f)); }
PP_DEVINL float gelu_fast_f(float x) {
  const float ax = __builtin_fabsf(x);
  const float t = __builtin_amdgcn_rcpf(__builtin_fmaf(ax, 0.3275911f * 0.70710678118654752440f, 1.0f));
  float p = __builtin_fmaf(t, 0.5f * 1.061405429f, 0.5f * -1.453152027f);
  p = __builtin_fmaf(t, p, 0.5f * 1.421413741f);
  p = __builtin_fmaf(t, p, 0.5f * -0.284496736f);
  p = __builtin_fmaf(t, p, 0.5f * 0.254829592f);
  const float q = p * t * __builtin_amdgcn_exp2f(x * x * (-0.5f * 1.44269504088896340736f));
  return __builtin_fmaf(-ax, q, __builtin_fmaxf(x, 0.f));
}

PP_DEVINL __amdgpu_buffer_rsrc_t make_rsrc(const void* base, uint32_t bytes) {
  return __builtin_amdgcn_make_buffer_rsrc(const_cast<void*>(base), 0, bytes, 0x00020000);
}
#define PP_OOB 0x80000000u

PP_DEVINL float wave_sum(float v) {
#pragma unroll
  for (int o = 32; o > 0; o >>= 1) v += __shfl_xor(v, o, 64);
  return v;
}
PP_DEVINL float wave_max(float v) {
#pragma unroll
  for (int o = 32; o > 0; o >>= 1) v = fmaxf(v, __shfl_xor(v, o, 64));
  return v;
}

#ifdef PP_LAB
inline int pp_lab_env(const char* name, int dflt) {
  const char* e = getenv(name);
  return e ? atoi(e) : dflt;
}
#else
constexpr int pp_lab_env(const char*, int dflt) { return dflt; }
#endif

void pp_set_last_error(const char* what, hipError_t e);
int pp_func_lds(const void* kern, int bytes, const char* what);
int pp_cu_count();
long long pp_l2_bytes();
struct CGChoice {
  int bm, splitk;
  int group_m = 1;
};
void pp_conv_gn_operand_bytes(const PPGemmArgs& a, int bm, long long* panel, long long* strip);
int pp_conv_gn_form(const PPGemmArgs& a, CGChoice* c);
int pp_conv_gn_run(const PPGemmArgs& a, const CGChoice& c, hipStream_t st);
#define PP_CHECK_LAUNCH(what)                         \
  do {                                                \
    hipError_t e__ = hipGetLastError();               \
    if (e__ != hipSuccess) {                          \
      pp_set_last_error(what, e__);                   \
      return PP_ERR_LAUNCH;                           \
    }                                                 \
  } while (0)
```

powerpaint_amd/engine.py:

```python
import ctypes as C
import enum
import math
import os
from dataclasses import dataclass
from typing import Dict, List, NamedTuple, Optional, Sequence, Tuple

import torch

from . import _lib as L

ALIGN = 256


def _align(x: int, a: int = ALIGN) -> int:
    return (x + a - 1) // a * a


def _lab_switch(name: str) -> bool:
    return not (os.environ.get("PP_LAB") == "1" and os.environ.get(name, "1") == "0")


GN_STATS_IN_EPILOGUE = _lab_switch("PP_GN_EPILOGUE")
GN_NEXT_IN_COMBINE = _lab_switch("PP_GN_NEXT")
FUSE_GN_CONV = _lab_switch("PP_FUSE_GN_CONV")
TWIN_PREFIX = _lab_switch("PP_TWIN")
FUSED_COMBINE = _lab_switch("PP_FUSED_COMBINE")
UPCONV_SUBPIX = _lab_switch("PP_UPCONV_SUBPIX")
UPCONV_SUBPIX_FROM = 1 if (os.environ.get("PP_LAB") == "1" and os.environ.get("PP_UPCONV_SUBPIX") == "2") else 2


def level_sizes(H: int, W: int, levels: int) -> List[Tuple[int, int]]:
    out = [(H, W)]
    for _ in range(levels - 1):
        h, w = out[-1]
        out.append(((h - 1) // 2 + 1, (w - 1) // 2 + 1))
    return out


class Arena:

    def __init__(self, nbytes: int = 0, device=None):
        self.dry = device is None
        self.size = nbytes
        if not self.dry:
            self.buf = torch.zeros(max(nbytes, ALIGN) + ALIGN, dtype=torch.uint8, device=device)
            skew = (-self.buf.data_ptr()) % ALIGN
            self.buf = self.buf[skew:skew + max(nbytes, ALIGN)]
            self.base = self.buf.data_ptr()
        else:
            self.buf = None
            self.base = 1 << 20
        self.off = 0
        self.peak = 0

    def alloc(self, nbytes: int) -> int:
        off = _align(self.off)
        self.off = off + nbytes
        self.peak = max(self.peak, self.off)
        if not self.dry and self.off > self.size:
            raise L.PPError(f"arena overflow: need {self.off} > {self.size}")
        return self.base + off

    def mark(self) -> int:
        return self.off

    def release(self, m: int):
        self.off = m

    def view(self, ptr: int, shape: Sequence[int], dtype: torch.dtype, strides: Optional[Sequence[int]] = None):
        esize = torch.empty((), dtype=dtype).element_size()
        off = ptr - self.base
        assert off % esize == 0
        typed = self.buf.view(dtype)
        if strides is None:
            n = 1
            for s in shape:
                n *= s
            return typed[off // esize: off // esize + n].view(*shape)
        return torch.as_strided(typed, tuple(shape), tuple(strides), off // esize)


class ParamPack:

    def __init__(self):
        self.items: List[Tuple[str, torch.Tensor]] = []
        self.offsets: Dict[str, int] = {}
        self.shapes: Dict[str, Tuple[torch.Size, torch.dtype]] = {}
        self.total = 0
        self.buf = None
        self.ptr: Dict[str, int] = {}
        self.version = 0

    def touch(self):
        self.version += 1

    def add(self, name: str, t: torch.Tensor, dtype: torch.dtype):
        assert name not in self.offsets, name
        t = t.detach().to(dtype).contiguous()
        off = _align(self.total)
        self.offsets[name] = off
        self.shapes[name] = (t.shape, dtype)
        self.total = off + t.numel() * t.element_size()
        self.items.append((name, t))

    def to_device(self, device, materialize: bool = True):
        self.buf = torch.zeros(_align(self.total) + ALIGN, dtype=torch.uint8, device=device)
        skew = (-self.buf.data_ptr()) % ALIGN
        self.buf = self.buf[skew:skew + _align(self.total)]
        base = self.buf.data_ptr()
        for name, t in self.items:
            off = self.offsets[name]
            if materialize and t.device.type != "meta":
                nb = t.numel() * t.element_size()
                self.buf[off:off + nb].copy_(t.view(-1).view(torch.uint8))
            self.ptr[name] = base + off
        self.items = []
        return self

    def regrow(self, keep: int):
        old = self.buf
        self.total = max(self.total, keep)
        buf = torch.zeros(_align(self.total) + ALIGN, dtype=torch.uint8, device=old.device)
        skew = (-buf.data_ptr()) % ALIGN
        buf = buf[skew:skew + _align(self.total)]
        buf[:keep].copy_(old[:keep])
        for name, t in self.items:
            off, nb = self.offsets[name], t.numel() * t.element_size()
            buf[off:off + nb].copy_(t.view(-1).view(torch.uint8))
        self.items = []
        self.buf = buf
        base = buf.data_ptr()
        self.ptr.clear()
        self.ptr.update({name: base + off for name, off in self.offsets.items()})
        self.touch()

    def forget(self, prefix: str, keep: int):
        for name in [n for n in self.offsets if n.startswith(prefix)]:
            assert self.offsets[name] >= keep, name
            del self.offsets[name], self.shapes[name]
            self.ptr.pop(name, None)
        self.total = keep

    def tensor(self, name: str) -> torch.Tensor:
        shape, dtype = self.shapes[name]
        off = self.offsets[name]
        n = 1
        for s in shape:
            n *= s
        es = torch.empty((), dtype=dtype).element_size()
        return self.buf[off:off + n * es].view(dtype).view(shape)


@dataclass
class Act:
    ptr: int
    B: int
    H: int
    W: int
    C: int
    producer: object = None
    dup_half: int = 0
    gn_filled: object = None

    @property
    def rows(self) -> int:
        return self.B * self.H * self.W

    @property
    def nbytes(self) -> int:
        return self.rows * self.C * 2


class Plan:

    def __init__(self):
        self.calls: List[Tuple] = []
        self.keep: List = []
        self.flops = 0.0
        self.flops_by_kind: Dict[str, float] = {}
        self.flops_skipped = 0.0

    def add(self, name: str, fn, *args):
        self.calls.append((fn, args, name))

    def count(self, kind: str, flops: float):
        self.flops += flops
        self.flops_by_kind[kind] = self.flops_by_kind.get(kind, 0.0) + flops

    def skip(self, flops: float):
        self.flops += flops
        self.flops_skipped += flops

    @property
    def flops_executed(self) -> float:
        return self.flops - self.flops_skipped

    def run(self, stream: int):
        for fn, args, name in self.calls:
            rc = fn(*args, stream)
            if rc != 0:
                L.check(rc, name)

    def run_timed(self, stream_obj) -> Dict[str, float]:
        evs = []
        s = stream_obj.cuda_stream
        for fn, args, name in self.calls:
            e0 = torch.cuda.Event(enable_timing=True)
            e1 = torch.cuda.Event(enable_timing=True)
            e0.record(stream_obj)
            rc = fn(*args, s)
            e1.record(stream_obj)
            if rc != 0:
                L.check(rc, name)
            evs.append((name, e0, e1))
        stream_obj.synchronize()
        out: Dict[str, float] = {}
        self.last_launch_ms = []
        for name, e0, e1 in evs:
            dt = e0.elapsed_time(e1)
            out[name] = out.get(name, 0.0) + dt
            self.last_launch_ms.append(dt)
        return out

    def describe(self, i: int) -> str:
        fn, args, name = self.calls[i]
        a = getattr(args[0], "_obj", None) if args else None
        if isinstance(a, L.PPGemmArgs):
            return (f"{name} M={a.M} N={a.N} K={a.K} {'conv' if a.x_mode else 'lin'}"
                    f"{' s2' if a.stride == 2 else ''}{' up' if a.up else ''}{' cat' if a.c2 else ''}"
                    f" gm={L.lib().pp_gemm_tile_group_m(C.byref(a))}")
        return name


class Builder:

    def __init__(self, arena: Arena, plan: Optional[Plan] = None, dtype: torch.dtype = torch.bfloat16):
        self.arena = arena
        self.plan = plan or Plan()
        self.lib = L.lib()
        self.dtype = dtype
        self.dt = L.dtype_code(dtype)
        self.gemm_tile = 0
        self.gemm_splitk = 0
        self.last_gemm = None
        self.gn_acc_base = 0
        self.gn_acc_cap = 0
        self.gn_acc_used = 0
        self.fault_ptr = 0

    def alloc(self, nbytes: int) -> int:
        return self.arena.alloc(nbytes)

    def new_act(self, B, H, W, Cc) -> Act:
        return Act(self.alloc(B * H * W * Cc * 2), B, H, W, Cc)

    def mark(self):
        return self.arena.mark()

    def release(self, m):
        self.arena.release(m)

    def _gemm(self, a: L.PPGemmArgs, name: str):
        if a.tile == 0:
            a.tile = self.gemm_tile
        if a.splitk == 0:
            a.splitk = self.gemm_splitk
        a.dtype = self.dt
        ws = self.lib.pp_gemm_workspace_bytes(C.byref(a))
        if ws:
            a.workspace = self.alloc(ws)
            if FUSED_COMBINE and self.gn_acc_cap:
                nctr = _align(self.lib.pp_gemm_combine_ctr_bytes(C.byref(a)), 8)
                if nctr and self.gn_acc_used + nctr <= self.gn_acc_cap:
                    a.tile_ctr = self.gn_acc_base + self.gn_acc_used
                    a.combine_fault = self.fault_ptr or None
                    self.gn_acc_used += nctr
        self.plan.keep.append(a)
        self.last_gemm = a
        a._arena_top = self.arena.off
        self.plan.add(name, self.lib.pp_gemm_bf16, C.byref(a))
        if a.subpix:
            self.plan.count(name, 4 * 2.0 * a.M * a.N * a.K)
            self.plan.skip(5 * 2.0 * a.M * a.N * a.K)
        else:
            self.plan.count(name, 2.0 * a.M * a.N * a.K)

    def linear(self, x: int, rows: int, K: int, w: int, N: int, bias: int = 0, ldx: Optional[int] = None,
               x2: int = 0, K2: int = 0, ldx2: int = 0, res1: int = 0, ldres1: int = 0, res2: int = 0,
               ldres2: int = 0, scale: float = 1.0, act: int = 0, out: int = 0, ldo: Optional[int] = None,
               rowvec: int = 0, ld_rowvec: int = 0, rows_per_batch: int = 0, out_vt: int = 0, vt_col0: int = 0,
               vt_ld: int = 0, out_f32: bool = False, row_stats_out: int = 0, ln_stats: int = 0, ln_colsum: int = 0,
               ln_tiles: int = 0, ln_dim: int = 0, ln_eps: float = 1e-5, name: str = "gemm", res1_wrap: int = 0,
               w_batch_stride: int = 0, vec_batch_stride: int = 0) -> int:
        n_out = N // 2 if act == L.PP_ACT_GEGLU else (vt_col0 if out_vt else N)
        if ldo is None:
            ldo = n_out
        if not out:
            out = self.alloc(rows * ldo * (4 if out_f32 else 2))
        m = self.mark()
        a = L.gemm_args(self.dt, rows, N, K, x, w, out, x2=x2, K2=K2, ldx=ldx, ldx2=ldx2, ldo=ldo, ldres1=ldres1, ldres2=ldres2,
                        rows_per_batch=rows_per_batch, scale=scale)
        a.bias, a.rowvec, a.ld_rowvec, a.res1, a.res2 = bias or None, rowvec or None, ld_rowvec, res1 or None, res2 or None
        a.w_batch_stride, a.vec_batch_stride, a.res1_wrap_rows = w_batch_stride, vec_batch_stride, res1_wrap
        a.act, a.out_f32 = act, int(out_f32)
        a.out_vt, a.vt_col0, a.vt_ld = out_vt or None, vt_col0, vt_ld
        a.row_stats_out = row_stats_out or None
        if ln_stats:
            a.ln_stats, a.ln_colsum, a.ln_tiles, a.ln_dim, a.ln_eps = ln_stats, ln_colsum, ln_tiles, ln_dim, ln_eps
        self._gemm(a, name)
        self.release(m)
        return out

    def conv3x3(self, x: Act, w: int, cout: int, bias: int = 0, stride: int = 1, up: bool = False,
                x2: Optional[Act] = None, rowvec: int = 0, res1: int = 0, res2: int = 0, scale: float = 1.0,
                out: Optional[Act] = None, x3: Optional[Act] = None, x4: Optional[Act] = None,
                name: str = "conv3x3", gn_in: Optional[Tuple[int, int, int, float, int]] = None, dup: bool = False,
                up_size: Optional[Tuple[int, int]] = None) -> Act:
        if gn_in is not None:
            gamma, beta, gb, eps, groups = gn_in
            acc = self._subscribe_gn_stats(x, x2, groups) if FUSE_GN_CONV else 0
            fused = None
            if acc:
                fused = (acc, gb, groups, eps)
            else:
                x, x2 = self.groupnorm(x, gamma, beta, eps, True, x2=x2, groups=groups), None
        else:
            fused = None
        c2 = x2.C if x2 is not None else 0
        ptr = lambda t: t.ptr if t is not None else None
        a = L.conv3x3_args(self.dt, x.B, x.H, x.W, x.C, cout, x.ptr, ptr(x2), c2, ptr(x3), x3.C if x3 is not None else 0,
                           ptr(x4), x4.C if x4 is not None else 0, stride, up, w=w, scale=scale, up_size=up_size)
        ho, wo = a.hout, a.wout
        if dup:
            assert out is None and gn_in is None
            out = self.new_act(2 * x.B, ho, wo, cout)
            out.dup_half = x.B
        if out is None:
            out = self.new_act(x.B, ho, wo, cout)
        m = self.mark()
        a.out, a.bias, a.rowvec, a.res1, a.res2 = out.ptr, bias or None, rowvec or None, res1 or None, res2 or None
        if dup:
            a.out_dup_rows = a.M
            if self.lib.pp_gemm_workspace_bytes(C.byref(a)):
                raise L.PPError("twin-prefix conv would run split-K; the caller must not request dup for this shape")
        if fused is not None:
            a.gn_in_acc, a.gn_in_gb, a.gn_in_groups, a.gn_in_eps, a.gn_in_silu = fused[0], fused[1], fused[2], fused[3], 1
            if not self.lib.pp_conv_gn_preferred(C.byref(a)):
                a.gn_in_acc, a.gn_in_gb, a.gn_in_groups, a.gn_in_silu = None, None, 0, 0
                gamma, beta, gb, eps, groups = gn_in
                self.release(m)
                xn = self._apply_in_producer_combine(x, fused[0], gamma, beta, eps, True, None) if x2 is None else None
                if xn is None:
                    xn = self.new_act(x.B, x.H, x.W, x.C + c2)
                    self.plan.add("groupnorm_apply", self.lib.pp_groupnorm_apply_acc, x.ptr, x.C,
                                  x2.ptr if x2 is not None else None, c2, x.B, x.H * x.W, groups, eps, gamma, beta, fused[0],
                                  1, xn.ptr, self.dt)
                m = self.mark()
                a.x1, a.x2, a.c1, a.c2 = xn.ptr, None, x.C + c2, 0
        self._gemm(a, name)
        out.producer = a
        self.release(m)
        return out

    def conv3x3_up_subpix(self, x: Act, wfold: int, cout: int, bias: int = 0, res2: int = 0, name: str = "conv3x3") -> Act:
        a = L.conv3x3_args(self.dt, x.B, x.H, x.W, x.C, cout, x.ptr, w=wfold)
        a.K, a.subpix = 4 * x.C, 1
        out = self.new_act(x.B, 2 * x.H, 2 * x.W, cout)
        a.out, a.bias, a.res2 = out.ptr, bias or None, res2 or None
        self._gemm(a, name)
        out.producer = a
        return out

    def groupnorm(self, x: Act, gamma: int, beta: int, eps: float, silu: bool, x2: Optional[Act] = None,
                  groups: int = 32, out: Optional[Act] = None) -> Act:
        c2 = x2.C if x2 is not None else 0
        Ct = x.C + c2
        hw = x.H * x.W
        out_given = out
        x2p = x2.ptr if x2 is not None else None
        acc = self._subscribe_gn_stats(x, x2, groups)
        if acc and x2 is None:
            fused = self._apply_in_producer_combine(x, acc, gamma, beta, eps, silu, out_given)
            if fused is not None:
                return fused
        if out is None:
            out = self.new_act(x.B, x.H, x.W, Ct)
        if acc:
            self.plan.add("groupnorm_apply", self.lib.pp_groupnorm_apply_acc, x.ptr, x.C, x2p, c2, x.B, hw, groups, eps,
                          gamma, beta, acc, int(silu), out.ptr, self.dt)
            return out
        m = self.mark()
        ws = self.alloc(self.lib.pp_groupnorm_workspace_bytes(x.B, hw, Ct))
        self.plan.add("groupnorm_stats", self.lib.pp_groupnorm_stats, x.ptr, x.C, x2p, c2, x.B, hw, groups, ws,
                      self.dt)
        self.plan.add("groupnorm_apply", self.lib.pp_groupnorm_apply, x.ptr, x.C, x2p, c2, x.B, hw, groups, eps,
                      gamma, beta, ws, int(silu), out.ptr, self.dt)
        self.release(m)
        return out

    def _apply_in_producer_combine(self, x: Act, acc: int, gamma: int, beta: int, eps: float, silu: bool,
                                   out: Optional[Act]) -> Optional[Act]:
        a = x.producer
        if not GN_NEXT_IN_COMBINE or a is None or not acc or not self.plan.calls or a.gn_next_out or \
                getattr(a, "_fused_ff", False):
            return None
        last = self.plan.calls[-1][1]
        if not last or getattr(last[0], "_obj", None) is not a:
            return None
        sub = 0 if a.gn_acc[0] == acc else 1 if a.gn_acc[1] == acc else -1
        if sub < 0 or not self.lib.pp_gemm_gn_next_ok(C.byref(a), sub):
            return None
        if out is None:
            self.arena.off = max(self.arena.off, getattr(a, "_arena_top", self.arena.off))
            out = self.new_act(x.B, x.H, x.W, x.C)
        elif out.ptr < self.arena.base + getattr(a, "_arena_top", 0):
            return None
        a.gn_next_out, a.gn_next_gamma, a.gn_next_beta = out.ptr, gamma, beta
        a.gn_next_eps, a.gn_next_silu, a.gn_next_sub = eps, int(silu), sub
        return out

    def _subscribe_gn_stats(self, x: Act, x2: Optional[Act], groups: int) -> int:
        if not (GN_STATS_IN_EPILOGUE and self.gn_acc_cap):
            return 0
        if x.gn_filled is not None or (x2 is not None and x2.gn_filled is not None):
            f = x.gn_filled
            return f[0] if (f is not None and x2 is not None and x2.gn_filled is f and f[1] == groups) else 0
        hw = x.H * x.W
        parts = [(x, 0)] + ([(x2, x.C)] if x2 is not None else [])
        Ct = x.C + (x2.C if x2 is not None else 0)
        if hw % 64 or Ct % groups or Ct // groups < 8:
            return 0
        for t, _ in parts:
            a = t.producer
            if a is None or (a.gn_acc[0] and a.gn_acc[1]):
                return 0
            rows = hw // 4 if a.subpix else hw
            rpb = a.rows_per_batch
            a.rows_per_batch = rows
            ok = self.lib.pp_gemm_gn_stats_ok(C.byref(a))
            a.rows_per_batch = rpb
            if not ok or (rpb not in (0, rows)):
                return 0
        nbytes = x.B * groups * 2 * 8
        if self.gn_acc_used + nbytes > self.gn_acc_cap:
            return 0
        acc = self.gn_acc_base + self.gn_acc_used
        self.gn_acc_used += nbytes
        for t, c0 in parts:
            a = t.producer
            k = 0 if not a.gn_acc[0] else 1
            a.rows_per_batch = hw // 4 if a.subpix else hw
            a.gn_acc[k], a.gn_cg[k], a.gn_c0[k], a.gn_groups[k] = acc, Ct // groups, c0, groups
            if t.dup_half:
                a.gn_dup_batch, a.gn_dup_mask = t.dup_half, a.gn_dup_mask | (1 << k)
        return acc

    def freeu(self, h: Act, sk: Act, bs: int, groups: int) -> Tuple[Act, Act]:
        assert (h.B, h.H, h.W) == (sk.B, sk.H, sk.W)
        Ct, nbytes, acc = h.C + sk.C, h.B * groups * 2 * 8, 0
        if GN_STATS_IN_EPILOGUE and self.gn_acc_cap and Ct % groups == 0 and self.gn_acc_used + nbytes <= self.gn_acc_cap:
            acc = self.gn_acc_base + self.gn_acc_used
            self.gn_acc_used += nbytes
        self.plan.add("freeu", self.lib.pp_freeu, h.ptr, h.ptr, h.C, sk.ptr, sk.ptr, sk.C, h.B, h.H, h.W, bs, acc or None,
                      groups, self.dt)
        filled = (acc, groups) if acc else None
        return (Act(h.ptr, h.B, h.H, h.W, h.C, gn_filled=filled), Act(sk.ptr, sk.B, sk.H, sk.W, sk.C, gn_filled=filled))

    def layernorm(self, x: int, rows: int, Cc: int, gamma: int, beta: int, eps: float = 1e-5, out: int = 0) -> int:
        out = out or self.alloc(rows * Cc * 2)
        self.plan.add("layernorm", self.lib.pp_layernorm, x, rows, Cc, gamma, beta, eps, out, self.dt)
        return out

    def attention(self, q: int, ldq: int, k: int, ldk: int, vt: int, ldvt: int, B: int, heads: int, nq: int,
                  nk: int, d: int, out: int = 0, ldo: int = 0, log2q: bool = False) -> int:
        Cc = heads * d
        if not out:
            out, ldo = self.alloc(B * nq * Cc * 2), Cc
        if log2q:
            self.plan.add("attention", self.lib.pp_attention_fwd_variant, q, ldq, k, ldk, vt, ldvt, out, ldo, B, heads, nq,
                          nk, d, float(d) ** -0.5, self.dt, L.PP_ATTN_PIPE_LOG2)
        else:
            self.plan.add("attention", self.lib.pp_attention_fwd, q, ldq, k, ldk, vt, ldvt, out, ldo, B, heads, nq, nk,
                          d, float(d) ** -0.5, self.dt)
        self.plan.count("attention", 4.0 * B * heads * nq * nk * d)
        return out

    def attention_tiled(self, q: int, ldq: int, k: int, ldk: int, vt: int, ldvt: int, B: int, heads: int, h: int, w: int,
                        nh: int, nw: int, d: int, out: int = 0, ldo: int = 0, log2q: bool = False) -> int:
        Cc, n = heads * d, h * w
        if not out:
            out, ldo = self.alloc(B * n * Cc * 2), Cc
        self.plan.add("attention", self.lib.pp_attention_fwd_tiled, q, ldq, k, ldk, vt, ldvt, out, ldo, B, heads, h, w, nh, nw,
                      d, float(d) ** -0.5, L.PP_ATTN_PIPE_LOG2 if log2q else L.PP_ATTN_AUTO, self.dt)
        self.plan.count("attention", 4.0 * B * heads * n * (n // (nh * nw)) * d)
        return out

    def ip_attn_add(self, q: int, ldq: int, k_ip: int, v_ip: int, o: int, ldo: int, B: int, heads: int, nq: int, nk: int,
                    d: int, scale, row_w: int = 0):
        if row_w:
            self.plan.add("ip_attn_add", self.lib.pp_ip_attn_add_masked, q, ldq, k_ip, v_ip, o, ldo, B, heads, nq, nk, d,
                          float(d) ** -0.5, scale, row_w, self.dt)
        else:
            self.plan.add("ip_attn_add", self.lib.pp_ip_attn_add, q, ldq, k_ip, v_ip, o, ldo, B, heads, nq, nk, d,
                          float(d) ** -0.5, scale, self.dt)
        self.plan.count("ip_attn_add", 4.0 * B * nq * nk * heads * d)

    def perceiver_attn(self, q: int, ldq: int, kv_x: int, ldkx: int, nx: int, kv_l: int, ldkl: int, nl: int, B: int, heads: int,
                       nq: int, out: int = 0) -> int:
        d = 64
        out = out or self.alloc(B * nq * heads * d * 2)
        self.plan.add("perceiver_attn", self.lib.pp_perceiver_attn, q, ldq, kv_x, ldkx, nx, kv_l or None, ldkl, nl, out,
                      heads * d, B, heads, nq, d, float(d) ** -0.5, self.dt)
        self.plan.count("perceiver_attn", 4.0 * B * heads * nq * (nx + nl) * d)
        return out

    def ff_fused(self, hs: int, rows: int, Cc: int, hw: int, w1: int, b1: int, cs1: int, ln_stats: int, ln_tiles: int,
                 w2: int, bias2: int, out: int, res1: int = 0, res1_wrap: int = 0, res2: int = 0, w2_kperm: bool = False):
        a = L.gemm_args(self.dt, rows, Cc, 4 * Cc, hs, w2, out, x2=hs, K2=Cc, rows_per_batch=hw)
        a.bias, a.res1, a.res2, a.res1_wrap_rows = bias2 or None, res1 or None, res2 or None, res1_wrap
        a.splitk = 1
        a._fused_ff = True
        self.plan.keep.append(a)
        self.last_gemm = a
        a._arena_top = self.arena.off
        self.plan.add("ff_fused", self.lib.pp_ff_fused, C.byref(a), w1, b1, cs1 or None, ln_stats or None, ln_tiles, 1e-5,
                      int(w2_kperm))
        self.plan.count("ff_fused", 2.0 * rows * 8 * Cc * Cc + 2.0 * rows * Cc * 5 * Cc)
        return a

    def add(self, a: int, b: int, out: int, n: int):
        self.plan.add("add", self.lib.pp_add_bf16, a, b, out, n, self.dt)


# ... 1211 lines not shown
```

powerpaint_amd/ops.py:

```python
import ctypes as C
from typing import Optional

import torch

from . import _lib as L

_DT = {torch.float32: 0, torch.bfloat16: 1, torch.float16: 2}


def _s():
    return torch.cuda.current_stream().cuda_stream


def _p(t: Optional[torch.Tensor]):
    return t.data_ptr() if t is not None else None


def _set_gn(a, gn, rows_per_batch):
    if not gn:
        return
    a.rows_per_batch = rows_per_batch
    for k, (acc, cg, c0, groups) in enumerate(gn):
        a.gn_acc[k], a.gn_cg[k], a.gn_c0[k], a.gn_groups[k] = acc.data_ptr(), cg, c0, groups


last_combine = {"fused": False, "ctr": None}
_fault_words = {}


def _fault_word(device) -> torch.Tensor:
    key = torch.device(device)
    if key not in _fault_words:
        _fault_words[key] = torch.zeros(1, dtype=torch.int32, device=device)
    return _fault_words[key]


def combine_faults(device) -> int:
    return int(_fault_word(device).item())


def _attach_combine(a, device, enable):
    last_combine["fused"], last_combine["ctr"] = False, None
    if enable is None or enable is False:
        return
    bound = ((a.M + 127) // 128) * ((a.N + 159) // 160) * 16
    if torch.is_tensor(enable):
        ctr = enable
        assert ctr.dtype == torch.int64 and ctr.numel() * 8 >= bound
    else:
        n = L.lib().pp_gemm_combine_ctr_bytes(C.byref(a))
        if enable == "force":
            n = max(n, bound)
        if not n:
            return
        ctr = torch.zeros(n // 8, dtype=torch.int64, device=device)
    a.tile_ctr, a.combine_fault = ctr.data_ptr(), _fault_word(device).data_ptr()
    last_combine["ctr"] = ctr
    last_combine["fused"] = bool(L.lib().pp_gemm_combine_fused(C.byref(a)))


def _norm_out(out, shape, like: torch.Tensor, what: str) -> torch.Tensor:
    if out is None:
        return torch.empty(*shape, dtype=like.dtype, device=like.device)
    if tuple(out.shape) != tuple(shape) or not out.is_contiguous() or out.dtype != like.dtype or out.device != like.device:
        raise L.PPError(f"{what}: `out` must be a contiguous {list(shape)} tensor of the inputs' format")
    return out


def _view2d(t, rows: int, cols: int, dtype, like: torch.Tensor, what: str) -> torch.Tensor:
    if (t.dim() != 2 or tuple(t.shape) != (rows, cols) or t.stride(1) != 1 or t.stride(0) < cols or t.dtype != dtype
            or t.device != like.device):
        raise L.PPError(f"{what}: must be a [{rows}, {cols}] row-major view (unit column stride) of the output format")
    return t


def _rows_in(t, cols: int, like: torch.Tensor, what: str) -> int:
    if t.dim() != 2 or t.shape[1] != cols or t.stride(1) != 1 or (t.shape[0] > 1 and t.stride(0) < cols) or t.dtype != like.dtype \
            or t.device != like.device:
        raise L.PPError(f"{what}: must be a [rows, {cols}] row-major view (unit column stride) of the inputs' format")
    return t.stride(0) if t.shape[0] > 1 else cols


def _exact(t, shape, dtype, like: torch.Tensor, what: str) -> torch.Tensor:
    if tuple(t.shape) != tuple(shape) or not t.is_contiguous() or t.dtype != dtype or t.device != like.device:
        raise L.PPError(f"{what}: must be a contiguous {list(shape)} tensor of {dtype}")
    return t


def _vt_window(t, nb: int, cols: int, rows: int, like: torch.Tensor, what: str) -> torch.Tensor:
    if (t.dim() != 3 or tuple(t.shape) != (nb, cols, rows) or t.stride(2) != 1 or t.dtype != like.dtype or t.device != like.device
            or t.stride(1) < rows or (nb > 1 and t.stride(0) != cols * t.stride(1))):
        raise L.PPError(f"{what}: must be a [{nb}, {cols}, {rows}] window of a contiguous [nb, cols, ld] buffer of the inputs' format")
    return t


def _nhwc_view(t, shape, like: torch.Tensor, what: str) -> torch.Tensor:
    B, H, W, Cc = shape
    bad = t.dim() != 4 or tuple(t.shape) != tuple(shape) or t.stride(3) != 1 or t.dtype != like.dtype or t.device != like.device
    if not bad:
        ld = t.stride(2) if W > 1 else (t.stride(1) if H > 1 else (t.stride(0) if B > 1 else Cc))
        bad = (ld < Cc or (W > 1 and H > 1 and t.stride(1) != W * ld) or (B > 1 and H * W > 1 and t.stride(0) != H * W * ld))
    if bad:
        raise L.PPError(f"{what}: must be a {list(shape)} NHWC view of the inputs' format with dense pixels (channel stride = ld)")
    return t


def _nhwc_ld(t, shape) -> int:
    B, H, W, Cc = shape
    return t.stride(2) if W > 1 else (t.stride(1) if H > 1 else (t.stride(0) if B > 1 else Cc))


def _res_ld(t, shape, like: torch.Tensor, what: str, rows_only: bool = False) -> int:
    if t is None:
        return shape[3]
    if t.dim() == 2:
        if t.shape[1] != shape[3] or t.stride(1) != 1 or t.dtype != like.dtype or t.device != like.device or \
                (not rows_only and t.shape[0] != shape[0] * shape[1] * shape[2]):
            raise L.PPError(f"{what}: must be [{shape[0] * shape[1] * shape[2]}, {shape[3]}] rows of the inputs' format")
        return t.stride(0) if t.shape[0] > 1 else shape[3]
    if rows_only:
        shape = tuple(t.shape[:3]) + (shape[3],) if t.dim() == 4 else shape
    _nhwc_view(t, shape, like, what)
    return _nhwc_ld(t, shape)


last_workspace = {"bytes": 0}


def _workspace(lib, a, device, workspace):
    ws = lib.pp_gemm_workspace_bytes(C.byref(a))
    last_workspace["bytes"] = ws
    if workspace is None:
        return torch.empty(max(ws, 4) // 4, dtype=torch.float32, device=device) if ws else None
    if (workspace.dtype != torch.float32 or not workspace.is_contiguous() or workspace.device != device
            or workspace.numel() * 4 < ws):
        raise L.PPError(f"`workspace` must be a contiguous fp32 tensor of at least {ws} bytes on the inputs' device")
    return workspace if ws else None


def groupnorm_apply_acc(x: torch.Tensor, acc: torch.Tensor, gamma, beta, eps: float, silu: bool, groups: int = 32,
                        x2=None, out: Optional[torch.Tensor] = None):
    B, H, W, C1 = x.shape
    C2 = x2.shape[3] if x2 is not None else 0
    y = _norm_out(out, (B, H, W, C1 + C2), x, "groupnorm_apply_acc")
    L.check(L.lib().pp_groupnorm_apply_acc(_p(x), C1, _p(x2), C2, B, H * W, groups, eps, _p(gamma), _p(beta), _p(acc),
                                           int(silu), _p(y), L.dtype_code(x.dtype), _s()), "pp_groupnorm_apply_acc")
    return y


def gemm(x: torch.Tensor, w: torch.Tensor, bias=None, x2=None, res1=None, res2=None, scale: float = 1.0, act: int = 0,
         rowvec=None, rows_per_batch: int = 0, out_f32: bool = False, vt_col0: int = 0, tile: int = 0,
         splitk: int = 0, tile_group_m: int = 0, row_stats: bool = False, ln_stats=None, ln_colsum=None, ln_dim: int = 0,
         ln_eps: float = 1e-5, gn=None, res1_wrap: int = 0, fuse_combine: bool = False, out=None, vt=None, stats=None,
         workspace=None):
    lib = L.lib()
    M, K1 = x.shape
    K2 = x2.shape[1] if x2 is not None else 0
    N = w.shape[-2]
    n_out = N // 2 if act == L.PP_ACT_GEGLU else (vt_col0 if vt_col0 else N)
    odt = torch.float32 if out_f32 else x.dtype
    if out is None:
        out = torch.empty(M, n_out, dtype=odt, device=x.device)
    else:
        _view2d(out, M, n_out, odt, x, "gemm: `out`")
    a = L.gemm_args(L.dtype_code(x.dtype), M, N, K1, _p(x), _p(w), _p(out), x2=_p(x2), K2=K2, ldx=x.stride(0),
                    ldx2=x2.stride(0) if x2 is not None else 0, ldo=out.stride(0) if M > 1 else n_out,
                    ldres1=res1.stride(0) if res1 is not None else 0,
                    ldres2=res2.stride(0) if res2 is not None else 0, rows_per_batch=rows_per_batch, scale=scale)
    if w.dim() == 3:
        a.w_batch_stride = w.stride(0)
        if bias is not None and bias.dim() == 2:
            a.vec_batch_stride = bias.stride(0)
    a.bias, a.rowvec, a.res1, a.res2 = _p(bias), _p(rowvec), _p(res1), _p(res2)
    a.ld_rowvec = rowvec.stride(0) if (rowvec is not None and rowvec.dim() == 2 and rowvec.shape[0] > 1) else 0
    a.res1_wrap_rows, a.act, a.out_f32 = res1_wrap, act, int(out_f32)
    if vt_col0:
        nb, ncols = M // rows_per_batch, N - vt_col0
        if vt is None:
            vt = torch.zeros(nb, ncols, rows_per_batch, dtype=x.dtype, device=x.device)
        elif (vt.dim() != 3 or tuple(vt.shape) != (nb, ncols, rows_per_batch) or vt.stride(2) != 1 or vt.dtype != x.dtype
              or vt.device != x.device or vt.stride(1) < rows_per_batch or vt.stride(0) != ncols * vt.stride(1)):
            raise L.PPError(f"gemm: `vt` must be a [{nb}, {ncols}, {rows_per_batch}] window of a contiguous [nb, cols, vt_ld] "
                            "buffer of the inputs' format")
        a.out_vt, a.vt_col0, a.vt_ld = _p(vt), vt_col0, vt.stride(1)
    elif vt is not None:
        raise L.PPError("gemm: `vt` without vt_col0")
    a.tile, a.splitk, a.tile_group_m = tile, splitk, tile_group_m
    _set_gn(a, gn, rows_per_batch)
    if row_stats:
        tn = (N + 159) // 160
        if stats is None:
            stats = torch.zeros(M, tn, 2, dtype=torch.float32, device=x.device)
        elif (tuple(stats.shape) != (M, tn, 2) or not stats.is_contiguous() or stats.dtype != torch.float32
              or stats.device != x.device):
            raise L.PPError(f"gemm: `stats` must be a contiguous [{M}, {tn}, 2] fp32 tensor")
        a.row_stats_out = _p(stats)
    elif stats is not None:
        raise L.PPError("gemm: `stats` without row_stats")
    if ln_stats is not None:
        a.ln_stats, a.ln_colsum, a.ln_tiles, a.ln_dim, a.ln_eps = _p(ln_stats), _p(ln_colsum), ln_stats.shape[1], ln_dim, ln_eps
    wsb = _workspace(lib, a, x.device, workspace)
    a.workspace = _p(wsb)
    _attach_combine(a, x.device, fuse_combine)
    L.check(lib.pp_gemm_bf16(C.byref(a), _s()), "pp_gemm_bf16")
    if row_stats:
        return out, stats
    return (out, vt) if vt_col0 else out


def gn_gamma_beta(gamma: torch.Tensor, beta: torch.Tensor) -> torch.Tensor:
    return torch.stack([gamma.float(), beta.float()], 1).contiguous()


def conv_gn_supported(x: torch.Tensor, cout: int, x2=None, x3=None, x4=None, groups: int = 32) -> bool:
    a = _conv_request(x, cout, 1, False, x2, x3, x4)
    a.gn_in_acc, a.gn_in_gb, a.gn_in_groups, a.gn_in_silu, a.gn_in_eps = 1, 1, groups, 1, 1e-5
    return bool(L.lib().pp_conv_gn_supported(C.byref(a)))


def conv_halo_routed(x: torch.Tensor, cout: int, x2=None, x3=None, x4=None, stride: int = 1, up: bool = False,
                     tile: int = 0, up_size=None) -> bool:
    a = _conv_request(x, cout, stride, up, x2, x3, x4, up_size)
    a.tile = tile
    return L.lib().pp_conv_gn_supported(C.byref(a)) == 2


def _conv_request(x, cout, stride, up, x2, x3, x4, up_size=None) -> L.PPGemmArgs:
    B, H, W, C1 = x.shape
    ch = lambda t: t.shape[3] if t is not None else 0
    return L.conv3x3_args(L.dtype_code(x.dtype), B, H, W, C1, cout, _p(x), _p(x2), ch(x2), _p(x3), ch(x3), _p(x4), ch(x4),
                          stride, up, up_size=up_size)


def conv3x3(x: torch.Tensor, w: torch.Tensor, bias=None, stride: int = 1, up: bool = False, x2=None, rowvec=None,
            res1=None, res2=None, scale: float = 1.0, tile: int = 0, splitk: int = 0, gn=None, x3=None, x4=None,
            gn_in=None, gn_next=None, dup: bool = False, gn_dup_mask: int = 0, res1_wrap: int = 0,
            fuse_combine: bool = False, out=None, workspace=None, ynext=None, up_size=None, tile_group_m: int = 0):
    lib = L.lib()
    B, C1, C2, cout = x.shape[0], x.shape[3], (x2.shape[3] if x2 is not None else 0), w.shape[0]
    a = _conv_request(x, cout, stride, up, x2, x3, x4, up_size)
    ho, wo = a.hout, a.wout
    oshape = (2 * B if dup else B, ho, wo, cout)
    if out is None:
        out = torch.empty(*oshape, dtype=x.dtype, device=x.device)
    else:
        a.ldo = _nhwc_ld(_nhwc_view(out, oshape, x, "conv3x3: `out`"), oshape)
    a.w, a.out, a.scale = _p(w), _p(out), scale
    a.bias, a.rowvec, a.res1, a.res2 = _p(bias), _p(rowvec), _p(res1), _p(res2)
    rshape = (B, ho, wo, cout)
    a.ldres1 = _res_ld(res1, rshape, x, "conv3x3: `res1`", rows_only=res1_wrap > 0)
    a.ldres2 = _res_ld(res2, rshape, x, "conv3x3: `res2`")
    if rowvec is not None and rowvec.dim() == 2 and rowvec.shape[0] > 1:
        a.ld_rowvec = rowvec.stride(0)
    a.res1_wrap_rows = res1_wrap
    if dup:
        a.out_dup_rows = a.M
        if gn_dup_mask:
            a.gn_dup_batch, a.gn_dup_mask = B, gn_dup_mask
    a.tile, a.splitk, a.tile_group_m = tile, splitk, tile_group_m
    _set_gn(a, gn, ho * wo)
    if gn_next is None and ynext is not None:
        raise L.PPError("conv3x3: `ynext` without gn_next")
    if gn_next is not None:
        g_, b_, eps_, silu_, sub_ = gn_next
        ynext = _norm_out(ynext, oshape, x, "conv3x3: `ynext`")
        a.gn_next_out, a.gn_next_gamma, a.gn_next_beta = _p(ynext), _p(g_), _p(b_)
        a.gn_next_eps, a.gn_next_silu, a.gn_next_sub = eps_, int(silu_), sub_
    if gn_in is not None:
        acc, gb, groups, eps = gn_in
        assert gb.dtype == torch.float32 and gb.shape == (C1 + C2, 2) and gb.is_contiguous()
        a.gn_in_acc, a.gn_in_gb, a.gn_in_groups, a.gn_in_silu, a.gn_in_eps = _p(acc), _p(gb), groups, 1, eps
    wsb = _workspace(lib, a, x.device, workspace)
    a.workspace = _p(wsb)
    if gn_next is not None and not lib.pp_gemm_gn_next_ok(C.byref(a), a.gn_next_sub):
        raise L.PPError("pp_gemm_gn_next_ok() = 0 for this launch (PP_ERR_UNSUPPORTED)")
    _attach_combine(a, x.device, fuse_combine)
    L.check(lib.pp_gemm_bf16(C.byref(a), _s()), "pp_gemm_bf16(conv)")
    return (out, ynext) if gn_next is not None else out


def upconv_fold(w: torch.Tensor) -> torch.Tensor:
    cout, cin = w.shape[0], w.shape[1] // 9
    assert w.is_contiguous() and w.shape[1] == 9 * cin
    out = torch.empty(4, cout, 4 * cin, dtype=w.dtype, device=w.device)
    L.check(L.lib().pp_upconv_fold(_p(w), cout, cin, L.dtype_code(w.dtype), _p(out), _s()), "pp_upconv_fold")
    return out


def upconv_subpix_supported(x: torch.Tensor, cout: int) -> int:
    B, H, W, C1 = x.shape
    return int(L.lib().pp_upconv_subpix_supported(B, H, W, C1, cout, L.dtype_code(x.dtype)))


def conv3x3_up_subpix(x: torch.Tensor, wfold: torch.Tensor, bias=None, rowvec=None, res1=None, res2=None, scale: float = 1.0,
                      tile: int = 0, splitk: int = 0, gn=None, out=None, workspace=None, tile_group_m: int = 0):
    B, H, W, C1 = x.shape
    cout = wfold.shape[1]
    assert tuple(wfold.shape) == (4, cout, 4 * C1) and wfold.is_contiguous()
    a = L.conv3x3_args(L.dtype_code(x.dtype), B, H, W, C1, cout, _p(x))
    a.K, a.subpix = 4 * C1, 1
    if out is None:
        out = torch.empty(B, 2 * H, 2 * W, cout, dtype=x.dtype, device=x.device)
    else:
        a.ldo = _nhwc_ld(_nhwc_view(out, (B, 2 * H, 2 * W, cout), x, "conv3x3_up_subpix: `out`"), (B, 2 * H, 2 * W, cout))
    a.w, a.out, a.scale = _p(wfold), _p(out), scale
    a.bias, a.rowvec, a.res1, a.res2 = _p(bias), _p(rowvec), _p(res1), _p(res2)
    a.ldres1 = _res_ld(res1, (B, 2 * H, 2 * W, cout), x, "conv3x3_up_subpix: `res1`")
    a.ldres2 = _res_ld(res2, (B, 2 * H, 2 * W, cout), x, "conv3x3_up_subpix: `res2`")
    if rowvec is not None and rowvec.dim() == 2 and rowvec.shape[0] > 1:
        a.ld_rowvec = rowvec.stride(0)
    a.tile, a.splitk, a.tile_group_m = tile, splitk, tile_group_m
    _set_gn(a, gn, H * W)
    a.workspace = _p(_workspace(L.lib(), a, x.device, workspace))
    L.check(L.lib().pp_gemm_bf16(C.byref(a), _s()), "pp_gemm_bf16(sub-pixel upsampling conv)")
    return out


def groupnorm(x: torch.Tensor, gamma, beta, eps: float, silu: bool, groups: int = 32, x2=None,
              out: Optional[torch.Tensor] = None):
    lib = L.lib()
    B, H, W, C1 = x.shape
    C2 = x2.shape[3] if x2 is not None else 0
    Ct = C1 + C2
    ws = torch.empty(lib.pp_groupnorm_workspace_bytes(B, H * W, Ct) // 4, dtype=torch.float32, device=x.device)
    y = _norm_out(out, (B, H, W, Ct), x, "groupnorm")
    dt = L.dtype_code(x.dtype)
    L.check(lib.pp_groupnorm_stats(_p(x), C1, _p(x2), C2, B, H * W, groups, _p(ws), dt, _s()), "pp_groupnorm_stats")
    L.check(lib.pp_groupnorm_apply(_p(x), C1, _p(x2), C2, B, H * W, groups, eps, _p(gamma), _p(beta), _p(ws),
                                   int(silu), _p(y), dt, _s()), "pp_groupnorm_apply")
    return y


def layernorm(x: torch.Tensor, gamma, beta, eps: float = 1e-5, out: Optional[torch.Tensor] = None):
    rows, Cc = x.shape
    y = _norm_out(out, (rows, Cc), x, "layernorm")
    L.check(L.lib().pp_layernorm(_p(x), rows, Cc, _p(gamma), _p(beta), eps, _p(y), L.dtype_code(x.dtype), _s()),
            "pp_layernorm")
    return y


def transpose_v(v: torch.Tensor, batch: int, nk: int, ldvt: Optional[int] = None):
    cols = v.shape[1]
    ldvt = ldvt or (nk + 7) // 8 * 8
    vt = torch.empty(batch, cols, ldvt, dtype=v.dtype, device=v.device)
    L.check(L.lib().pp_transpose_v(_p(v), v.stride(0), batch, nk, cols, _p(vt), ldvt, _s()), "pp_transpose_v")
    return vt


def _attn_out(out, ldo, rows: int, cols: int, like: torch.Tensor) -> torch.Tensor:
    if out is None:
        return torch.empty(rows, ldo or cols, dtype=like.dtype, device=like.device)[:, :cols]
    if (tuple(out.shape) != (rows, cols) or out.stride(1) != 1 or out.dtype != like.dtype or out.device != like.device
            or (ldo is not None and ldo != out.stride(0))):
        raise L.PPError(f"attention: `out` must be a [{rows}, {cols}] row-major view of the inputs' format (row stride = ldo)")
    return out


def attention_small(q: torch.Tensor, k: torch.Tensor, v: torch.Tensor, batch: int, heads: int, nq: int, nk: int,
                    causal: bool = False, scale: Optional[float] = None, out: Optional[torch.Tensor] = None,
                    ldo: Optional[int] = None):
    d = 64
    o = _attn_out(out, ldo, batch * nq, heads * d, q)
    L.check(L.lib().pp_attention_small(_p(q), q.stride(0), _p(k), k.stride(0), _p(v), v.stride(0), _p(o), o.stride(0),
                                       batch, heads, nq, nk, d, scale if scale is not None else d ** -0.5, int(causal),
                                       L.dtype_code(q.dtype), _s()), "pp_attention_small")
    return o


def perceiver_attention(q: torch.Tensor, kv_x: torch.Tensor, kv_l: Optional[torch.Tensor], batch: int, heads: int, nq: int,
                        scale: Optional[float] = None, out: Optional[torch.Tensor] = None, ldo: Optional[int] = None):
    d = 64
    o = _attn_out(out, ldo, batch * nq, heads * d, q)
    nx, nl = kv_x.shape[0] // batch, (kv_l.shape[0] // batch if kv_l is not None else 0)
    L.check(L.lib().pp_perceiver_attn(_p(q), q.stride(0), _p(kv_x), kv_x.stride(0), nx, _p(kv_l),
                                      kv_l.stride(0) if kv_l is not None else 0, nl, _p(o), o.stride(0), batch, heads, nq, d,
                                      scale if scale is not None else d ** -0.5, L.dtype_code(q.dtype), _s()),
            "pp_perceiver_attn")
    return o


def softmax_rows(s: torch.Tensor, scale: float = 1.0, dtype=torch.bfloat16):
    rows, n = s.shape
    p = torch.empty(rows, n, dtype=dtype, device=s.device)
    L.check(L.lib().pp_softmax_rows(_p(s), s.stride(0), rows, n, float(scale), _p(p), n, L.dtype_code(dtype), _s()),
            "pp_softmax_rows")
    return p


def attention(q: torch.Tensor, k: torch.Tensor, vt: torch.Tensor, batch: int, heads: int, nq: int, nk: int, d: int,
              scale: Optional[float] = None, variant: int = L.PP_ATTN_AUTO, out: Optional[torch.Tensor] = None,
              ldo: Optional[int] = None):
    o = _attn_out(out, ldo, batch * nq, heads * d, q)
    L.check(L.lib().pp_attention_fwd_variant(_p(q), q.stride(0), _p(k), k.stride(0), _p(vt), vt.stride(1), _p(o),
                                             o.stride(0), batch, heads, nq, nk, d,
                                             scale if scale is not None else d ** -0.5, L.dtype_code(q.dtype),
                                             int(variant), _s()), "pp_attention_fwd")
    return o


def attention_tiled(q: torch.Tensor, k: torch.Tensor, vt: torch.Tensor, batch: int, heads: int, h: int, w: int, nh: int,
                    nw: int, d: int, scale: Optional[float] = None, variant: int = L.PP_ATTN_AUTO,
                    out: Optional[torch.Tensor] = None, ldo: Optional[int] = None):
    o = _attn_out(out, ldo, batch * h * w, heads * d, q)
    L.check(L.lib().pp_attention_fwd_tiled(_p(q), q.stride(0), _p(k), k.stride(0), _p(vt), vt.stride(1), _p(o), o.stride(0),
                                           batch, heads, h, w, nh, nw, d, scale if scale is not None else d ** -0.5,
                                           int(variant), L.dtype_code(q.dtype), _s()), "pp_attention_fwd_tiled")
    return o


def xattn_fold(k: torch.Tensor, vt: torch.Tensor, batch: int, nctx: int, heads: int, wq: torch.Tensor, wo: torch.Tensor,
               q_colsum=None, q_bias=None, scale: Optional[float] = None, kperm=False, gt=None, gcs=None, gbias=None,
               ht=None):
    c = wq.shape[0]
    dev, dt = k.device, k.dtype
    if k.dim() != 2 or k.shape[0] != batch * nctx or k.shape[1] < c or k.stride(1) != 1 or (k.shape[0] > 1 and k.stride(0) < c):
        raise L.PPError(f"xattn_fold: `k` must be [{batch * nctx}, >= {c}] rows with unit column stride")
    if (vt.dim() != 3 or vt.shape[0] != batch or vt.shape[1] != c or vt.shape[2] < nctx or vt.stride(2) != 1 or vt.dtype != dt
            or vt.stride(1) < nctx or (batch > 1 and vt.stride(0) != c * vt.stride(1))):
        raise L.PPError(f"xattn_fold: `vt` must be a [{batch}, {c}, >= {nctx}] window of a contiguous [batch, c, ldvt] buffer")
    for w_, nm in ((wq, "wq"), (wo, "wo")):
        if tuple(w_.shape) != (c, c) or not w_.is_contiguous() or w_.dtype != dt:
            raise L.PPError(f"xattn_fold: `{nm}` must be a contiguous [{c}, {c}] matrix of the inputs' format")
    n = heads * 80
    gt = torch.empty(batch, n, c, dtype=dt, device=dev) if gt is None else _exact(gt, (batch, n, c), dt, k, "xattn_fold: `gt`")
    ht = torch.empty(batch, c, n, dtype=dt, device=dev) if ht is None else _exact(ht, (batch, c, n), dt, k, "xattn_fold: `ht`")
    gcs = torch.empty(batch, n, dtype=torch.float32, device=dev) if gcs is None else \
        _exact(gcs, (batch, n), torch.float32, k, "xattn_fold: `gcs`")
    gb = torch.empty(batch, n, dtype=torch.float32, device=dev) if gbias is None else \
        _exact(gbias, (batch, n), torch.float32, k, "xattn_fold: `gbias`")
    L.check(L.lib().pp_xattn_fold(_p(k), k.stride(0) if k.shape[0] > 1 else k.shape[1], _p(vt), vt.stride(1), batch, nctx, heads, c, _p(wq), _p(q_colsum),
                                  _p(q_bias), _p(wo), scale if scale is not None else (c // heads) ** -0.5, _p(gt),
                                  _p(gcs), _p(gb), _p(ht), int(kperm), L.dtype_code(dt), _s()), "pp_xattn_fold")
    return gt, gcs, gb, ht


def xattn_block(x: torch.Tensor, folded, bias_o=None, res=None, ln_stats=None, ln_eps: float = 1e-5,
                rows_per_batch: int = 0, row_stats=False, twin: bool = False, pre_w=None, pre_b=None,
                ln_fold: bool = False, out=None):
    gt, gcs, gb, ht = folded
    wrap = x.shape[0] if twin else 0
    M, c = x.shape[0] * (2 if twin else 1), x.shape[1]
    ldx = _rows_in(x, c, x, "xattn_block: `x`")
    ldres = _rows_in(res, c, x, "xattn_block: `res`") if res is not None else 0
    if res is not None and res.shape[0] != x.shape[0]:
        raise L.PPError("xattn_block: `res` must have the rows of `x`")
    nb = M // (rows_per_batch or M)
    _exact(gt, (nb, 640, c), x.dtype, x, "xattn_block: folded gt")
    _exact(ht, (nb, c, 640), x.dtype, x, "xattn_block: folded ht")
    _exact(gcs, (nb, 640), torch.float32, x, "xattn_block: folded gcs")
    _exact(gb, (nb, 640), torch.float32, x, "xattn_block: folded gbias")
    out = torch.empty(M, c, dtype=x.dtype, device=x.device) if out is None else _view2d(out, M, c, x.dtype, x, "xattn_block: `out`")
    if torch.is_tensor(row_stats):
        st = _exact(row_stats, (M, c // 160, 2), torch.float32, x, "xattn_block: `row_stats`")
        row_stats = True
    else:
        st = torch.zeros(M, c // 160, 2, dtype=torch.float32, device=x.device) if row_stats else None
    tiles = ln_stats.shape[1] if ln_stats is not None else (c // 160 if (pre_w is not None and ln_fold) else 0)
    L.check(L.lib().pp_xattn_block(_p(x), ldx, _p(res), ldres, _p(ln_stats),
                                   tiles, ln_eps, _p(gt), _p(gcs), _p(gb), _p(ht),
                                   _p(bias_o), _p(out), out.stride(0) if M > 1 else c, _p(st), M, c, rows_per_batch or M, wrap, _p(pre_w), _p(pre_b),
                                   L.dtype_code(x.dtype), _s()), "pp_xattn_block")
    return (out, st) if row_stats else out


def ff_fused(hs: torch.Tensor, w1: torch.Tensor, b1: torch.Tensor, w2kp: torch.Tensor, bias2=None, cs1=None, ln_stats=None,
             ln_eps: float = 1e-5, res1=None, res2=None, res1_wrap: int = 0, rows_per_batch: int = 0, gn=None,
             w2_kperm: bool = True, scale: float = 1.0, out=None):
    M, Cc = hs.shape
    ldx = _rows_in(hs, Cc, hs, "ff_fused: `hs`")
    ld1 = _rows_in(res1, Cc, hs, "ff_fused: `res1`") if res1 is not None else 0
    ld2 = _rows_in(res2, Cc, hs, "ff_fused: `res2`") if res2 is not None else 0
    if res1 is not None and res1.shape[0] != (res1_wrap or M):
        raise L.PPError(f"ff_fused: `res1` must have {res1_wrap or M} rows")
    if res2 is not None and res2.shape[0] != M:
        raise L.PPError(f"ff_fused: `res2` must have {M} rows")
    if tuple(w1.shape) != (8 * Cc, Cc) or not w1.is_contiguous() or tuple(w2kp.shape) != (Cc, 5 * Cc) or not w2kp.is_contiguous():
        raise L.PPError("ff_fused: `w1` / `w2kp` must be contiguous [2560, 320] / [320, 1600] matrices")
    out = torch.empty(M, Cc, dtype=hs.dtype, device=hs.device) if out is None else _view2d(out, M, Cc, hs.dtype, hs, "ff_fused: `out`")
    a = L.gemm_args(L.dtype_code(hs.dtype), M, Cc, 4 * Cc, _p(hs), _p(w2kp), _p(out), x2=_p(hs), K2=Cc, ldx2=ldx,
                    ldo=out.stride(0) if M > 1 else Cc, ldres1=ld1, ldres2=ld2, rows_per_batch=rows_per_batch, scale=scale)
    a.bias, a.res1, a.res2, a.res1_wrap_rows = _p(bias2), _p(res1), _p(res2), res1_wrap
    _set_gn(a, gn, rows_per_batch)
    L.check(L.lib().pp_ff_fused(C.byref(a), _p(w1), _p(b1), _p(cs1), _p(ln_stats),
                                ln_stats.shape[1] if ln_stats is not None else 0, ln_eps, int(w2_kperm), _s()), "pp_ff_fused")
    return out


def gn_conv3x3_smallcout(x, acc, gamma, beta, eps: float, w, bias, groups: int = 32):
    B, H, W, Cin = x.shape
    out = torch.empty(B, w.shape[0], H, W, dtype=torch.float32, device=x.device)
    L.check(L.lib().pp_gn_conv3x3_smallcout(_p(x), B, H, W, Cin, groups, eps, _p(gamma), _p(beta), _p(acc), _p(w), _p(bias),
                                            w.shape[0], _p(out), L.dtype_code(x.dtype), _s()), "pp_gn_conv3x3_smallcout")
    return out


def conv3x3_direct(x, w, bias, stride: int = 1, silu: bool = False, add=None):
    B, H, W, Cin = x.shape
    cout = w.shape[3]
    ho, wo = (H - 1) // stride + 1, (W - 1) // stride + 1
    out = torch.empty(B, ho, wo, cout, dtype=x.dtype, device=x.device)
    L.check(L.lib().pp_conv3x3_direct(_p(x), B, H, W, Cin, _p(w), _p(bias), cout, stride, int(silu), _p(add), _p(out),
                                      L.dtype_code(x.dtype), _s()), "pp_conv3x3_direct")
    return out


def conv3x3_smallcout(x, w, bias):
    B, H, W, Cin = x.shape
    out = torch.empty(B, w.shape[0], H, W, dtype=torch.float32, device=x.device)
    L.check(L.lib().pp_conv3x3_smallcout(_p(x), B, H, W, Cin, _p(w), _p(bias), w.shape[0], _p(out),
                                         L.dtype_code(x.dtype), _s()), "pp_conv3x3_smallcout")
    return out


def nchw_to_nhwc(src: torch.Tensor, batch: Optional[int] = None, ldc: Optional[int] = None, c0: int = 0, dst=None,
                 dtype=torch.bfloat16):
    B, Cc, H, W = src.shape
    nb = batch or B
    ldc = ldc or Cc
    if dst is None:
        dst = torch.zeros(nb, H, W, ldc, dtype=dtype, device=src.device)
    src = src.contiguous()
    L.check(L.lib().pp_nchw_to_nhwc(_p(src), _DT[src.dtype], nb, Cc, H * W, B if nb != B else 0, _p(dst), ldc, c0,
                                    L.dtype_code(dst.dtype), _s()), "pp_nchw_to_nhwc")
    return dst


def nhwc_to_nchw(src: torch.Tensor, dtype=torch.float32):
    B, H, W, Cc = src.shape
    dst = torch.empty(B, Cc, H, W, dtype=dtype, device=src.device)
    L.check(L.lib().pp_nhwc_to_nchw(_p(src), B, Cc, H * W, _p(dst), _DT[dtype], L.dtype_code(src.dtype), _s()),
            "pp_nhwc_to_nchw")
    return dst


def vit_patchify(src: torch.Tensor, patch: int, out: Optional[torch.Tensor] = None, dtype=torch.bfloat16):
    B, Cc, H, W = src.shape
    if Cc != 3:
        raise L.PPError("vit_patchify: src must be [B, 3, H, W]")
    rows = B * (H // patch) * (W // patch)
    if out is None:
        out = torch.empty(rows, (3 * patch * patch + 63) // 64 * 64, dtype=dtype, device=src.device)
    elif out.dim() != 2 or out.shape[0] != rows or out.stride(1) != 1 or out.stride(0) < out.shape[1] or out.device != src.device:
        raise L.PPError(f"vit_patchify: `out` must be a [{rows}, cols] row-major 16-bit view on the source's device")
    src = src.contiguous()
    L.check(L.lib().pp_vit_patchify(_p(src), _DT[src.dtype], B, H, W, patch, _p(out), out.shape[1], out.stride(0), L.dtype_code(out.dtype),
                                    _s()), "pp_vit_patchify")
    return out


def vit_embed_ln(patches: torch.Tensor, class_embedding: torch.Tensor, pos: torch.Tensor, batch: int, gamma, beta,
                 eps: float = 1e-5, out: Optional[torch.Tensor] = None):
    Cc = patches.shape[1]
    npatch = patches.shape[0] // batch
    ldp = _rows_in(patches, Cc, patches, "vit_embed_ln: `patches`")
    if patches.shape[0] != batch * npatch or tuple(pos.shape) != (npatch + 1, Cc) or class_embedding.numel() != Cc or \
            pos.dtype != patches.dtype or class_embedding.dtype != patches.dtype:
        raise L.PPError("vit_embed_ln: patches [batch * np, C], class_embedding [C], pos [np + 1, C] of one 16-bit format")
    y = _norm_out(out, (batch * (npatch + 1), Cc), patches, "vit_embed_ln")
    L.check(L.lib().pp_vit_embed_ln(_p(patches), ldp, _p(class_embedding.contiguous()), _p(pos.contiguous()), batch, npatch, Cc,
                                    _p(gamma), _p(beta), eps, _p(y), L.dtype_code(patches.dtype), _s()), "pp_vit_embed_ln")
    return y


def add(a: torch.Tensor, b: torch.Tensor):
    out = torch.empty_like(a)
    L.check(L.lib().pp_add_bf16(_p(a), _p(b), _p(out), a.numel(), L.dtype_code(a.dtype), _s()), "pp_add_bf16")
    return out


def freeu(hidden: torch.Tensor, skip: torch.Tensor, b: float, s: float, acc: Optional[torch.Tensor] = None,
          groups: int = 32, inplace: bool = False):
    B, H, W, Ch = hidden.shape
    ho, so = (hidden, skip) if inplace else (torch.empty_like(hidden), torch.empty_like(skip))
    bs = torch.tensor([b, s], dtype=torch.float32, device=hidden.device)
    L.check(L.lib().pp_freeu(_p(hidden), _p(ho), Ch, _p(skip), _p(so), skip.shape[3], B, H, W, _p(bs), _p(acc), groups,
                             L.dtype_code(hidden.dtype), _s()), "pp_freeu")
    return ho, so


def timestep_embedding(t: torch.Tensor, rows: int, dim: int):
    out = torch.empty(rows, dim, dtype=torch.float32, device=t.device)
    L.check(L.lib().pp_timestep_embedding(_p(t), rows, dim, _p(out), _s()), "pp_timestep_embedding")
    return out
# ... 109 lines not shown
```

Baseline: 9.350 images/s.

## Add optional four-stage weight ring to raw conv_gn loops with per-launch LDS sizing

Adds a templated stage count to the conv+GroupNorm kernel, so the raw (no input-norm) ping-pong and sub-pixel loops can keep a four-deep weight ring with a longer prefetch lookahead, selected per shape class through a runtime mask. The LDS layout is reworked: halo buffers are sized from the actual tile halo rather than a fixed maximum, and the dynamic LDS request is computed per launch. Sub-pixel launches also stop loading halo rows they never read, and out-of-range strips go to a dump slot. The shipped class mask is zero, so the four-stage path stays off unless enabled through a lab environment switch; the smaller LDS request and the skipped loads do apply by default.

Result: no change. 9.345 images/s (-0.1%).

```diff
diff --git a/include/pp_hip.h b/include/pp_hip.h
--- a/include/pp_hip.h
+++ b/include/pp_hip.h
@@ -108,6 +108,8 @@
 int pp_gemm_gn_stats_ok(const PPGemmArgs* args);
 int pp_conv_gn_supported(const PPGemmArgs* args);
 int pp_conv_gn_preferred(const PPGemmArgs* args);
+int pp_conv_gn_set_ring(int class_mask);
+int pp_conv_gn_ring(const PPGemmArgs* args);
 int pp_upconv_subpix_supported(int batch, int h, int w, int cin, int cout, int dtype);
 int pp_upconv_subpix_supported_to(int batch, int h, int w, int hout, int wout, int cin, int cout, int dtype);
 int pp_upconv_fold(const void* w, int cout, int cin, int dtype, void* out, void* stream);
diff --git a/powerpaint_amd/_lib.py b/powerpaint_amd/_lib.py
--- a/powerpaint_amd/_lib.py
+++ b/powerpaint_amd/_lib.py
@@ -112,6 +112,8 @@
     "pp_gemm_gn_stats_ok": (C.c_int, [C.POINTER(PPGemmArgs)]),
     "pp_conv_gn_supported": (C.c_int, [C.POINTER(PPGemmArgs)]),
     "pp_conv_gn_preferred": (C.c_int, [C.POINTER(PPGemmArgs)]),
+    "pp_conv_gn_set_ring": (C.c_int, [C.c_int]),
+    "pp_conv_gn_ring": (C.c_int, [C.POINTER(PPGemmArgs)]),
     "pp_gemm_gn_next_ok": (C.c_int, [C.POINTER(PPGemmArgs), C.c_int]),
     "pp_upconv_subpix_supported": (C.c_int, [C.c_int] * 6),
     "pp_upconv_subpix_supported_to": (C.c_int, [C.c_int] * 8),
diff --git a/powerpaint_amd/csrc/conv_gn.hip b/powerpaint_amd/csrc/conv_gn.hip
--- a/powerpaint_amd/csrc/conv_gn.hip
+++ b/powerpaint_amd/csrc/conv_gn.hip
@@ -1,3 +1,5 @@
+#include <algorithm>
+#include <atomic>
 #include <type_traits>
 #include <utility>
 
@@ -13,22 +15,44 @@
 constexpr int CG_WP = 3;
 constexpr int CG_HPW_MAX = 6;
 constexpr int CG_HALO_PX = 384;
-constexpr int CG_HALO = CG_HALO_PX * 128;
 constexpr int CG_WST = CG_BN * 128;
-constexpr int CG_WOFF = 2 * CG_HALO;
-constexpr int CG_TAB = CG_WOFF + 3 * CG_WST;
-constexpr int CG_T_STATS = CG_TAB;
-constexpr int CG_T_ZERO = CG_TAB + 256;
-constexpr int CG_T_GB = CG_TAB + 1024;
-constexpr int CG_T_SCSH = CG_TAB + 3072;
-constexpr int CG_LDS = CG_TAB + 3584;
-static_assert(CG_LDS <= 160 * 1024, "LDS budget");
+constexpr int CG_LDS_MAX = 160 * 1024;
+constexpr int CG_TAB_NORM = 3584;
+constexpr int CG_T_STATS = 0;
+constexpr int CG_T_GB = 1024;
+constexpr int CG_T_SCSH = 3072;
+constexpr int CG_TAB_RAW = 2048;
+constexpr int CG_T_DUMP = 1024;
+constexpr int cg_tab(bool norm) { return norm ? CG_TAB_NORM : CG_TAB_RAW; }
+constexpr int cg_t_zero(bool norm) { return norm ? 256 : 0; }
+static_assert(CG_TAB_NORM + 2 * CG_HALO_PX * 128 + 3 * CG_WST <= CG_LDS_MAX, "LDS budget");
+
+constexpr int cg_nxt(int hpw, bool gb, int tt) {
+  const int nh = tt > 2 ? 0 : (2 * tt + 2 <= hpw ? 2 : 2 * tt + 1 <= hpw ? 1 : 0);
+  return nh + ((gb && tt == 0) ? 1 : 0);
+}
+constexpr int cg_vcount(int T, int NS, int hpw, bool gb, int t, bool halo_due) {
+  int n = 0;
+  for (int back = 0; back <= NS - 2; ++back) {
+    const int nx = cg_nxt(hpw, gb, ((t - back) % T + T) % T);
+    if (halo_due && nx > 0) return n;
+    n += nx;
+    if (back == NS - 2) break;
+    n += CG_WP;
+  }
+  return n;
+}
+static_assert(cg_vcount(9, 3, 5, true, 0, false) == 0 + CG_WP + 3 && cg_vcount(9, 3, 5, true, 1, false) == 3 + CG_WP + 2, "3-stage count");
+static_assert(cg_vcount(4, 3, 5, false, 3, true) == CG_WP && cg_vcount(4, 3, 5, false, 0, false) == 0 + CG_WP + 2, "3-stage count");
+static_assert(cg_vcount(9, 4, 5, false, 5, false) == 2 * CG_WP && cg_vcount(9, 4, 5, false, 1, false) == 0 + CG_WP + 2 + CG_WP + 2, "4-stage count");
+static_assert(cg_vcount(4, 4, 5, false, 3, true) == CG_WP && cg_vcount(4, 4, 3, false, 3, true) == 2 * CG_WP, "4-stage count");
 
 struct CGDerived {
   int tiles_m, tiles_n, group_m;
   int nch1, nch;
   int ntail3, ntail;
   int hp;
+  int hbytes;
   int cg;
   float inv_cg;
 };
@@ -38,7 +62,7 @@
 template <int N, class F>
 PP_DEVINL void cg_static_for(F&& f) { cg_static_for_impl(std::make_integer_sequence<int, N>{}, f); }
 
-template <int BM, int HPW, bool PP, int NMODE, int EDT>
+template <int BM, int HPW, bool PP, int NMODE, int EDT, int NS>
 __global__ void __launch_bounds__(CG_T, 2) pp_conv_gn_kernel(const PPGemmArgs a, const CGDerived d) {
   using E = E16<EDT>;
   typedef typename E::v8 v8_t;
@@ -49,12 +73,16 @@
   constexpr bool NORM = NMODE != 2 && !SUBPIX;
   constexpr bool NREAD = NMODE == 0 || NMODE == 3;
   static_assert(HPW >= 2 && HPW <= CG_HPW_MAX, "halo strips per wave");
+  static_assert(NS == 3 || (NS == 4 && PP && (NMODE == 2 || SUBPIX)), "a fourth stage: the raw ping-pong loops only");
+  constexpr int LOOK = NS - 1;
+  constexpr int CG_T_ZERO = cg_t_zero(NORM);
   constexpr int XP2 = BM / 64;
   constexpr int P2 = XP2 + CG_WP;
   constexpr int ST2 = BM * 128;
+  constexpr int WOFF2 = 3 * ST2;
   constexpr int EPI_ROWS = 64, EPI_LD = BN * 4 + 16;
   constexpr int RS_OFF = EPI_ROWS * EPI_LD + BM * 8;
-  static_assert(3 * ST2 <= 2 * CG_HALO, "tail stages live in the halo buffers");
+  static_assert(WOFF2 + 3 * CG_WST <= CG_LDS_MAX, "the tail's three (X, weight) stages");
   static_assert(MI * 16 <= EPI_ROWS && EPI_ROWS % (MI * 16) == 0, "wave rows vs epilogue pass");
 
   extern __shared__ __attribute__((aligned(16))) char smem[];
@@ -86,6 +114,9 @@
   const int y0 = (m_blk - bimg * HW) / Wd;
   const int ctot = a.c1 + a.c2;
   const uint32_t wbytes = (uint32_t)a.N * (uint32_t)a.K * 2u;
+  const int hbytes = d.hbytes;
+  constexpr int hoff0 = cg_tab(NORM);
+  const int woff = hoff0 + 2 * hbytes;
   const void* const wmat = SUBPIX ? (const void*)((const char*)a.w + (size_t)par * wbytes) : a.w;
 
   const int lrow = lane >> 3;
@@ -105,7 +136,8 @@
     const int hp = (wave + 8 * j) * 8 + lrow;
     const int hr = hp / Wd, hx = hp - hr * Wd;
     const int iy = y0 + hr - 1;
-    hpix[j] = (hp < d.hp && iy >= 0 && iy < Hd) ? (a.up ? bimg * HWs + (iy >> 1) * a.win + (hx >> 1) : bimg * HW + iy * Wd + hx) : -1;
+    const bool unread = SUBPIX && hr == (pa ? 0 : BM / Wd + 1);
+    hpix[j] = (hp < d.hp && iy >= 0 && iy < Hd && !unread) ? (a.up ? bimg * HWs + (iy >> 1) * a.win + (hx >> 1) : bimg * HW + iy * Wd + hx) : -1;
   }
   const int r16 = lane & 15, g = lane >> 4;
   const int fsw = r16 & 7;
@@ -161,7 +193,7 @@
       asm volatile("s_waitcnt lgkmcnt(0)" ::: "memory");
     };
     auto norm_piece = [&](int hbuf, int j) __attribute__((always_inline)) {
-      char* p = smem + hbuf * CG_HALO + (wave + 8 * j) * 1024 + lane * 16;
+      char* p = smem + hoff0 + hbuf * hbytes + (wave + 8 * j) * 1024 + lane * 16;
       if (hpix[j] >= 0) {
         const u32x4_t v = *reinterpret_cast<const u32x4_t*>(p);
         float r[8];
@@ -215,24 +247,25 @@
     };
     auto issue_halo_piece = [&](int hbuf, int j) __attribute__((always_inline)) {
       const int vo = hpix[j] >= 0 ? (hpix[j] * hcsrc + kslot * 8) * 2 : (int)PP_OOB;
-      __builtin_amdgcn_raw_ptr_buffer_load_lds(rs_h, (cg_lds_t)(smem + hbuf * CG_HALO + (wave + 8 * j) * 1024), 16, vo,
-                                               hsoff, 0, 0);
+      const int strip = wave + 8 * j;
+      const int lo = (!NORM && strip * 8 >= d.hp) ? CG_T_DUMP : hoff0 + hbuf * hbytes + strip * 1024;
+      __builtin_amdgcn_raw_ptr_buffer_load_lds(rs_h, (cg_lds_t)(smem + lo), 16, vo, hsoff, 0, 0);
     };
     auto issue_w_piece = [&](const __amdgpu_buffer_rsrc_t rs, int stage, int i, int sow) __attribute__((always_inline)) {
       const int vo = vw[i], lo = wlds[i];
-      __builtin_amdgcn_raw_ptr_buffer_load_lds(rs, (cg_lds_t)(smem + CG_WOFF + stage * CG_WST + lo), 16, vo, sow, 0, 0);
+      __builtin_amdgcn_raw_ptr_buffer_load_lds(rs, (cg_lds_t)(smem + woff + stage * CG_WST + lo), 16, vo, sow, 0, 0);
     };
 
     {
       const __amdgpu_buffer_rsrc_t rsw = make_rsrc(wmat, wbytes);
 #pragma unroll
-      for (int i = 0; i < CG_WP; ++i) issue_w_piece(rsw, 0, i, (0 * ctot + ch_b * 64) * 2);
-#pragma unroll
-      for (int i = 0; i < CG_WP; ++i) issue_w_piece(rsw, 1, i, (1 * ctot + ch_b * 64) * 2);
+      for (int s = 0; s < LOOK; ++s)
+#pragma unroll
+        for (int i = 0; i < CG_WP; ++i) issue_w_piece(rsw, s, i, (s * ctot + ch_b * 64) * 2);
       halo_source(ch_b, true);
 #pragma unroll
       for (int j = 0; j < CG_HPW; ++j) issue_halo_piece(0, j);
-      issue_gb(ch_b, 0, true);
+      if constexpr (NORM) issue_gb(ch_b, 0, true);
     }
     if (NORM && tid < a.gn_in_groups) {
       const long long* ap = reinterpret_cast<const long long*>(a.gn_in_acc) + ((size_t)bimg * a.gn_in_groups + tid) * 2;
@@ -265,21 +298,20 @@
         halo_source(c + 1, nxt);
         const __amdgpu_buffer_rsrc_t rsw_same = make_rsrc(wmat, wbytes);
         const __amdgpu_buffer_rsrc_t rsw_next = make_rsrc(wmat, nxt ? wbytes : 0u);
-        const int hoff = hb * CG_HALO;
+        const int hoff = hoff0 + hb * hbytes;
         const int hbn = hb ^ 1;
         int Wl = Wd;
         asm volatile("" : "+s"(Wl));
 
         cg_static_for<4>([&](auto TT) __attribute__((always_inline)) {
           constexpr int t = decltype(TT)::value;
-          constexpr auto NXT = [](int tt) constexpr { return tt > 2 ? 0 : (2 * tt + 2 <= CG_HPW ? 2 : 2 * tt + 1 <= CG_HPW ? 1 : 0); };
-          constexpr int NX = NXT(t);
-          const int st_w = st == 0 ? 2 : st - 1;
-          const __amdgpu_buffer_rsrc_t rsw = t + 2 <= 3 ? rsw_same : rsw_next;
-          const int sow = t + 2 <= 3 ? ((t + 2) * ctot + c * 64) * 2 : ((t + 2 - 4) * ctot + (c + 1) * 64) * 2;
+          constexpr int NX = cg_nxt(CG_HPW, false, t);
+          const int st_w = st == 0 ? NS - 1 : st - 1;
+          const __amdgpu_buffer_rsrc_t rsw = t + LOOK <= 3 ? rsw_same : rsw_next;
+          const int sow = t + LOOK <= 3 ? ((t + LOOK) * ctot + c * 64) * 2 : ((t + LOOK - 4) * ctot + (c + 1) * 64) * 2;
 
           asm volatile("s_barrier" ::: "memory");
-          const char* ws = smem + CG_WOFF + st * CG_WST;
+          const char* ws = smem + woff + st * CG_WST;
           const int hp0 = rt0 + tap00 + (t / 2) * Wl + (t % 2);
           const int xbase = hoff + (hp0 << 7) + ((g ^ (hp0 & 7)) << 4);
           const unsigned em = t % 2 == 0 ? em0 : em1;
@@ -308,48 +340,47 @@
                 __builtin_amdgcn_sched_barrier(0);
               }
           }
-          constexpr int V = (t == 3 ? 0 : NXT((t + 3) % 4)) + CG_WP + NX;
+          constexpr int V = cg_vcount(4, NS, CG_HPW, false, t, t == 3);
           asm volatile("s_waitcnt vmcnt(%0) lgkmcnt(0)\n\ts_barrier" ::"n"(V) : "memory");
           __builtin_amdgcn_sched_barrier(0);
           __builtin_amdgcn_s_setprio(1);
           mfma_all(wf, xf);
           __builtin_amdgcn_s_setprio(0);
           __builtin_amdgcn_sched_barrier(0);
-          st = st == 2 ? 0 : st + 1;
+          st = st == NS - 1 ? 0 : st + 1;
         });
         hb ^= 1;
       }
     } else {
+      int st = 0;
   #pragma unroll 1
       for (int c = ch_b; c < ch_e; ++c) {
         const bool nxt = c + 1 < ch_e;
         halo_source(c + 1, nxt);
         const __amdgpu_buffer_rsrc_t rsw_same = make_rsrc(wmat, wbytes);
         const __amdgpu_buffer_rsrc_t rsw_next = make_rsrc(wmat, nxt ? wbytes : 0u);
-        const int hoff = hb * CG_HALO;
+        const int hoff = hoff0 + hb * hbytes;
         const int hbn = hb ^ 1;
         int Wl = Wd;
         asm volatile("" : "+s"(Wl));
 
         cg_static_for<9>([&](auto TT) __attribute__((always_inline)) {
           constexpr int t = decltype(TT)::value;
-          constexpr int st_r = t % 3, st_w = (t + 2) % 3;
-          constexpr auto NXT = [](int tt) constexpr {
-            const int nh = tt > 2 ? 0 : (2 * tt + 2 <= CG_HPW ? 2 : 2 * tt + 1 <= CG_HPW ? 1 : 0);
-            return nh + (tt == 0 ? 1 : 0);
-          };
+          const int st_r = NS == 3 ? t % 3 : st, st_w = NS == 3 ? (t + 2) % 3 : (st == 0 ? NS - 1 : st - 1);
+          constexpr auto NXT = [](int tt) constexpr { return cg_nxt(CG_HPW, NORM, tt); };
           constexpr int NX = NXT(t);
-          const __amdgpu_buffer_rsrc_t rsw = t + 2 <= 8 ? rsw_same : rsw_next;
-          const int sow = t + 2 <= 8 ? ((t + 2) * ctot + c * 64) * 2 : ((t + 2 - 9) * ctot + (c + 1) * 64) * 2;
+          const __amdgpu_buffer_rsrc_t rsw = t + LOOK <= 8 ? rsw_same : rsw_next;
+          const int sow = t + LOOK <= 8 ? ((t + LOOK) * ctot + c * 64) * 2 : ((t + LOOK - 9) * ctot + (c + 1) * 64) * 2;
 
           if constexpr (PP) {
             asm volatile("s_barrier" ::: "memory");
           } else {
+            static_assert(PP || NS == 3, "the lock-step loop has three stages");
             constexpr int V = NXT((t + 7) % 9) + CG_WP + NXT((t + 8) % 9);
             asm volatile("s_waitcnt vmcnt(%0) lgkmcnt(0)\n\ts_barrier" ::"n"(V) : "memory");
           }
           constexpr bool NT = NORM && t >= 3 && t - 3 < CG_HPW;
-          char* const np = smem + hbn * CG_HALO + (wave + 8 * (NT ? t - 3 : 0)) * 1024 + lane * 16;
+          char* const np = smem + hoff0 + hbn * hbytes + (wave + 8 * (NT ? t - 3 : 0)) * 1024 + lane * 16;
           u32x4_t nv = {0u, 0u, 0u, 0u};
           f32x4_t ss0 = {0.f, 0.f, 0.f, 0.f}, ss1 = {0.f, 0.f, 0.f, 0.f};
           if constexpr (NT) {
@@ -362,7 +393,7 @@
             }
             if constexpr (NREAD) __builtin_amdgcn_sched_barrier(0);
           }
-          const char* ws = smem + CG_WOFF + st_r * CG_WST;
+          const char* ws = smem + woff + st_r * CG_WST;
           const int hp0 = rt0 + (t / 3) * Wl + (t % 3) - 1;
           const int xbase = hoff + (hp0 << 7) + ((g ^ (hp0 & 7)) << 4);
           v8_t wf[2][NI], xf[2][MI];
@@ -387,13 +418,14 @@
               if (((k + 1) * NR + NPC) / (NPC + 1) == r + 1) {
                 __builtin_amdgcn_sched_barrier(0);
                 if (k < CG_WP) issue_w_piece(rsw, st_w, k < CG_WP ? k : 0, sow);
-                else if (t == 0 && k == NPC - 1) issue_gb(c + 1, hbn, nxt);
+                else if (NORM && t == 0 && k == NPC - 1) issue_gb(c + 1, hbn, nxt);
                 else issue_halo_piece(hbn, 2 * t + (k - CG_WP < 2 ? k - CG_WP : 0));
                 __builtin_amdgcn_sched_barrier(0);
               }
           }
           if constexpr (PP) {
-            constexpr int V = NXT((t + 8) % 9) + CG_WP + NX;
+            constexpr int V = cg_vcount(9, NS, CG_HPW, NORM, t, false);
+            static_assert(NS != 3 || V == NXT((t + 8) % 9) + CG_WP + NX, "the 3-stage count");
             asm volatile("s_waitcnt vmcnt(%0) lgkmcnt(0)\n\ts_barrier" ::"n"(V) : "memory");
           }
           __builtin_amdgcn_sched_barrier(0);
@@ -454,6 +486,7 @@
           }
           if constexpr (NMODE != 3) __builtin_amdgcn_s_setprio(0);
           __builtin_amdgcn_sched_barrier(0);
+          if constexpr (NS != 3) st = st == NS - 1 ? 0 : st + 1;
         });
         hb ^= 1;
       }
@@ -484,7 +517,7 @@
 #pragma unroll
       for (int i = 0; i < CG_WP; ++i) {
         const int vo = vw[i], lo = wlds[i];
-        __builtin_amdgcn_raw_ptr_buffer_load_lds(rsw, (cg_lds_t)(smem + CG_WOFF + stage * CG_WST + lo), 16, vo, sow, 0, 0);
+        __builtin_amdgcn_raw_ptr_buffer_load_lds(rsw, (cg_lds_t)(smem + WOFF2 + stage * CG_WST + lo), 16, vo, sow, 0, 0);
       }
     };
     issue2(tk_b, 0);
@@ -498,7 +531,7 @@
       if (nstage >= 3) nstage -= 3;
       issue2(kt + 2, nstage);
       const char* xs = smem + stage * ST2;
-      const char* ws = smem + CG_WOFF + stage * CG_WST;
+      const char* ws = smem + WOFF2 + stage * CG_WST;
       v8_t wf[2][NI], xf[2][MI];
 #pragma unroll
       for (int ks = 0; ks < 2; ++ks) {
@@ -635,7 +668,7 @@
     gn_flush(a, slots, m_blk, n_blk, ncols, tid);
   }
   if (splitk && a.tile_ctr) {
-    static_assert(fc_lds_bytes(BM) <= CG_LDS, "fused combine staging must fit in the kernel's LDS");
+    static_assert(fc_lds_bytes(BM) <= CG_LDS_MAX, "fused combine staging (cg_lds_bytes asks for at least this much)");
     splitk_fused_combine<BM, T, EDT>(a, smem, m_blk, n_blk, blockIdx.x, blockIdx.y, splits, tid);
   }
 }
@@ -729,10 +762,40 @@
   return c;
 }
 
-template <int BM, int HPW, bool PP, int NMODE, int EDT>
+bool cg_ring_fits(const PPGemmArgs& a, int bm) {
+  return CG_TAB_RAW + 2 * (bm + 2 * a.wout) * 128 + 4 * CG_WST <= CG_LDS_MAX;
+}
+int cg_ring_class(const PPGemmArgs& a, int bm) {
+  if (a.subpix) return 8;
+  if (bm == 256 && a.wout == 16) return 1;
+  if (bm == 128 && a.wout == 32) return 2;
+  if (bm == 128 && a.wout == 64) return 4;
+  return 16;
+}
+constexpr int CG_RING_SHIP = 0;
+std::atomic<int> cg_ring_mask{-1};
+int cg_ring(const PPGemmArgs& a, int bm) {
+  if (a.gn_in_acc || !cg_ring_fits(a, bm)) return 3;
+  const int m = cg_ring_mask.load(std::memory_order_relaxed);
+  return ((m < 0 ? CG_RING_SHIP : m) & cg_ring_class(a, bm)) ? 4 : 3;
+}
+
+template <int BM, bool NORM>
+int cg_lds_bytes(const PPGemmArgs& a, int hbytes, int ns) {
+  int b = cg_tab(NORM) + 2 * hbytes + ns * CG_WST;
+  if (a.c3 + a.c4 > 0) b = std::max(b, 3 * (BM * 128 + CG_WST));
+  b = std::max(b, 64 * (CG_BN * 4 + 16) + BM * 8 + 2 * GN_SLOTS * 2 * 8);
+  return std::max(b, fc_lds_bytes(BM));
+}
+
+template <int BM, int HPW, bool PP, int NMODE, int EDT, int NS = 3>
 int cg_launch(const PPGemmArgs& a, int splitk, int group_m, hipStream_t st) {
-  auto kern = pp_conv_gn_kernel<BM, HPW, PP, NMODE, EDT>;
-  if (pp_func_lds(reinterpret_cast<const void*>(kern), CG_LDS, "hipFuncSetAttribute(conv_gn)") != PP_OK) return PP_ERR_LAUNCH;
+  auto kern = pp_conv_gn_kernel<BM, HPW, PP, NMODE, EDT, NS>;
+  constexpr bool NORM = NMODE != 2 && NMODE != 4;
+  const int hbytes = NORM ? HPW * 8 * 1024 : (BM + 2 * a.wout) * 128;
+  const int lds = cg_lds_bytes<BM, NORM>(a, hbytes, NS);
+  if (lds > CG_LDS_MAX || (BM + 2 * a.wout) > HPW * 64) return PP_ERR_UNSUPPORTED;
+  if (pp_func_lds(reinterpret_cast<const void*>(kern), lds, "hipFuncSetAttribute(conv_gn)") != PP_OK) return PP_ERR_LAUNCH;
   CGDerived d;
   d.tiles_m = a.M / BM;
   d.tiles_n = (a.N + CG_BN - 1) / CG_BN;
@@ -742,16 +805,30 @@
   d.ntail3 = a.c3 / 64;
   d.ntail = (a.c3 + a.c4) / 64;
   d.hp = BM + 2 * a.wout;
+  d.hbytes = hbytes;
   d.cg = a.gn_in_groups > 0 ? (a.c1 + a.c2) / a.gn_in_groups : 1;
   d.inv_cg = 1.0f / (float)d.cg;
-  hipLaunchKernelGGL(kern, dim3(d.tiles_m * d.tiles_n * (NMODE == 4 ? 4 : 1), splitk, 1), dim3(CG_T), CG_LDS, st, a, d);
+  hipLaunchKernelGGL(kern, dim3(d.tiles_m * d.tiles_n * (NMODE == 4 ? 4 : 1), splitk, 1), dim3(CG_T), lds, st, a, d);
   PP_CHECK_LAUNCH("pp_conv_gn_kernel");
   return PP_OK;
 }
 
 template <int BM, bool PP, int NMODE, int EDT>
-int cg_launch_hpw(const PPGemmArgs& a, int splitk, int group_m, hipStream_t st) {
+int cg_launch_hpw(const PPGemmArgs& a, int splitk, int group_m, int ring, hipStream_t st) {
   const int need = (BM + 2 * a.wout + 63) / 64;
+  constexpr bool R4 = PP && (NMODE == 2 || NMODE == 4);
+  if constexpr (R4) {
+    if (ring == 4 && need <= 5) {
+      if constexpr (BM == 256) return cg_launch<256, 5, PP, NMODE, EDT, 4>(a, splitk, group_m, st);
+      else if constexpr (BM == 128) {
+        if (need <= 3) return cg_launch<128, 3, PP, NMODE, EDT, 4>(a, splitk, group_m, st);
+        if (need <= 4) return cg_launch<128, 4, PP, NMODE, EDT, 4>(a, splitk, group_m, st);
+      } else {
+        if (need <= 2) return cg_launch<64, 2, PP, NMODE, EDT, 4>(a, splitk, group_m, st);
+        if (need <= 3) return cg_launch<64, 3, PP, NMODE, EDT, 4>(a, splitk, group_m, st);
+      }
+    }
+  }
   if constexpr (BM == 256) {
     if (need <= 5) return cg_launch<256, 5, PP, NMODE, EDT>(a, splitk, group_m, st);
     return cg_launch<256, 6, PP, NMODE, EDT>(a, splitk, group_m, st);
@@ -772,10 +849,10 @@
   if (!pp || nm != 1) {
 #define CG_CASE(BM_)                                                                        \
     case BM_:                                                                               \
-      if (!pp) return cg_launch_hpw<BM_, false, 1, EDT>(a, c.splitk, c.group_m, st);                   \
-      if (nm == 0) return cg_launch_hpw<BM_, true, 0, EDT>(a, c.splitk, c.group_m, st);                \
-      if (nm == 2) return cg_launch_hpw<BM_, true, 2, EDT>(a, c.splitk, c.group_m, st);                \
-      return cg_launch_hpw<BM_, true, 3, EDT>(a, c.splitk, c.group_m, st);
+      if (!pp) return cg_launch_hpw<BM_, false, 1, EDT>(a, c.splitk, c.group_m, c.ring, st);                   \
+      if (nm == 0) return cg_launch_hpw<BM_, true, 0, EDT>(a, c.splitk, c.group_m, c.ring, st);                \
+      if (nm == 2) return cg_launch_hpw<BM_, true, 2, EDT>(a, c.splitk, c.group_m, c.ring, st);                \
+      return cg_launch_hpw<BM_, true, 3, EDT>(a, c.splitk, c.group_m, c.ring, st);
     switch (c.bm) {
       CG_CASE(256)
       CG_CASE(128)
@@ -787,22 +864,22 @@
 #endif
   if (a.subpix) {
     switch (c.bm) {
-      case 256: return cg_launch_hpw<256, true, 4, EDT>(a, 1, c.group_m, st);
-      case 128: return cg_launch_hpw<128, true, 4, EDT>(a, 1, c.group_m, st);
-      default: return cg_launch_hpw<64, true, 4, EDT>(a, 1, c.group_m, st);
+      case 256: return cg_launch_hpw<256, true, 4, EDT>(a, 1, c.group_m, c.ring, st);
+      case 128: return cg_launch_hpw<128, true, 4, EDT>(a, 1, c.group_m, c.ring, st);
+      default: return cg_launch_hpw<64, true, 4, EDT>(a, 1, c.group_m, c.ring, st);
     }
   }
   if (!a.gn_in_acc) {
     switch (c.bm) {
-      case 256: return cg_launch_hpw<256, true, 2, EDT>(a, c.splitk, c.group_m, st);
-      case 128: return cg_launch_hpw<128, true, 2, EDT>(a, c.splitk, c.group_m, st);
-      default: return cg_launch_hpw<64, true, 2, EDT>(a, c.splitk, c.group_m, st);
+      case 256: return cg_launch_hpw<256, true, 2, EDT>(a, c.splitk, c.group_m, c.ring, st);
+      case 128: return cg_launch_hpw<128, true, 2, EDT>(a, c.splitk, c.group_m, c.ring, st);
+      default: return cg_launch_hpw<64, true, 2, EDT>(a, c.splitk, c.group_m, c.ring, st);
     }
   }
   switch (c.bm) {
-    case 256: return cg_launch_hpw<256, true, 1, EDT>(a, c.splitk, c.group_m, st);
-    case 128: return cg_launch_hpw<128, true, 1, EDT>(a, c.splitk, c.group_m, st);
-    default: return cg_launch_hpw<64, true, 1, EDT>(a, c.splitk, c.group_m, st);
+    case 256: return cg_launch_hpw<256, true, 1, EDT>(a, c.splitk, c.group_m, c.ring, st);
+    case 128: return cg_launch_hpw<128, true, 1, EDT>(a, c.splitk, c.group_m, c.ring, st);
+    default: return cg_launch_hpw<64, true, 1, EDT>(a, c.splitk, c.group_m, c.ring, st);
   }
 }
 
@@ -813,6 +890,7 @@
   if (a.subpix) {
     if (!cg_subpix_ok(a)) return PP_ERR_UNSUPPORTED;
     *c = cg_choose_subpix(a);
+    c->ring = cg_ring(a, c->bm);
     return 1;
   }
   if (a.gn_in_acc) {
@@ -821,6 +899,7 @@
     return 0;
   }
   *c = cg_choose(a);
+  c->ring = cg_ring(a, c->bm);
   return 1;
 }
 void pp_conv_gn_operand_bytes(const PPGemmArgs& a, int bm, long long* panel, long long* strip) {
@@ -830,7 +909,20 @@
 }
 int pp_conv_gn_run(const PPGemmArgs& a, const CGChoice& c, hipStream_t st) {
   if (c.splitk > 1 && !a.workspace) return PP_ERR_WORKSPACE;
-  return a.dtype == PP_DT_F16 ? cg_dispatch<PP_DT_F16>(a, c, st) : cg_dispatch<PP_DT_BF16>(a, c, st);
+  CGChoice cc = c;
+  cc.ring = cg_ring(a, c.bm);
+  return a.dtype == PP_DT_F16 ? cg_dispatch<PP_DT_F16>(a, cc, st) : cg_dispatch<PP_DT_BF16>(a, cc, st);
+}
+
+extern "C" int pp_conv_gn_set_ring(int class_mask) {
+  if (class_mask < -1 || class_mask > 31) return PP_ERR_BAD_ARG;
+  cg_ring_mask.store(class_mask, std::memory_order_relaxed);
+  return PP_OK;
+}
+extern "C" int pp_conv_gn_ring(const PPGemmArgs* args) {
+  if (!args) return 0;
+  CGChoice c{0, 1};
+  return pp_conv_gn_form(*args, &c) == 1 ? c.ring : 0;
 }
 
 extern "C" int pp_conv_gn_supported(const PPGemmArgs* args) {
diff --git a/powerpaint_amd/csrc/pp_common.h b/powerpaint_amd/csrc/pp_common.h
--- a/powerpaint_amd/csrc/pp_common.h
+++ b/powerpaint_amd/csrc/pp_common.h
@@ -119,6 +119,7 @@
 struct CGChoice {
   int bm, splitk;
   int group_m = 1;
+  int ring = 3;
 };
 void pp_conv_gn_operand_bytes(const PPGemmArgs& a, int bm, long long* panel, long long* strip);
 int pp_conv_gn_form(const PPGemmArgs& a, CGChoice* c);
diff --git a/powerpaint_amd/engine.py b/powerpaint_amd/engine.py
--- a/powerpaint_amd/engine.py
+++ b/powerpaint_amd/engine.py
@@ -27,6 +27,8 @@
 FUSED_COMBINE = _lab_switch("PP_FUSED_COMBINE")
 UPCONV_SUBPIX = _lab_switch("PP_UPCONV_SUBPIX")
 UPCONV_SUBPIX_FROM = 1 if (os.environ.get("PP_LAB") == "1" and os.environ.get("PP_UPCONV_SUBPIX") == "2") else 2
+if os.environ.get("PP_LAB") == "1" and os.environ.get("PP_CONV_RING"):
+    L.check(L.lib().pp_conv_gn_set_ring(int(os.environ["PP_CONV_RING"])), "pp_conv_gn_set_ring")
 
 
 def level_sizes(H: int, W: int, levels: int) -> List[Tuple[int, int]]:
@@ -226,9 +228,10 @@
         fn, args, name = self.calls[i]
         a = getattr(args[0], "_obj", None) if args else None
         if isinstance(a, L.PPGemmArgs):
+            ring = L.lib().pp_conv_gn_ring(C.byref(a))
             return (f"{name} M={a.M} N={a.N} K={a.K} {'conv' if a.x_mode else 'lin'}"
                     f"{' s2' if a.stride == 2 else ''}{' up' if a.up else ''}{' cat' if a.c2 else ''}"
-                    f" gm={L.lib().pp_gemm_tile_group_m(C.byref(a))}")
+                    f" gm={L.lib().pp_gemm_tile_group_m(C.byref(a))}{f' ring={ring}' if ring else ''}")
         return name
 
 
diff --git a/powerpaint_amd/ops.py b/powerpaint_amd/ops.py
--- a/powerpaint_amd/ops.py
+++ b/powerpaint_amd/ops.py
@@ -279,6 +279,13 @@
     return (out, ynext) if gn_next is not None else out
 
 
+CONV_RING_CLASSES = {"w16_256": 1, "w32_128": 2, "w64_128": 4, "subpix": 8, "other": 16}
+
+
+def set_conv_ring(class_mask: int = -1) -> None:
+    L.check(L.lib().pp_conv_gn_set_ring(int(class_mask)), "pp_conv_gn_set_ring")
+
+
 def upconv_fold(w: torch.Tensor) -> torch.Tensor:
     cout, cin = w.shape[0], w.shape[1] // 9
     assert w.is_contiguous() and w.shape[1] == 9 * cin
```
